# ml-unito/PartitionedLS.jl

Measured on AMD Instinct MI355X. Metric: sign-pattern NNLS solves/sec (whole node); fp64 obj gap vs ref, higher is better.
Workload: dtype f64

## Files before the change

### partitionedls.jl_amd/csrc/ctx.h

```cpp
#pragma once
#include "common.h"
#include <chrono>
#include <functional>
#include <vector>

namespace partls {

bool runtime_gone();
struct NoCopy {
    NoCopy() = default;
    NoCopy(const NoCopy &) = delete;
    NoCopy &operator=(const NoCopy &) = delete;
};

struct DevBuf : NoCopy {
    void *p = nullptr;
    size_t bytes = 0;
    ~DevBuf() { release(); }
    hipError_t ensure(size_t b)
    {
        if (b <= bytes && p) return hipSuccess;
        if (p) { hipError_t e = hipFree(p); p = nullptr; bytes = 0; if (e != hipSuccess) return e; }
        hipError_t e = hipMalloc(&p, b ? b : 8);
        if (e == hipSuccess) bytes = b;
        return e;
    }
    void release() { if (p && !runtime_gone()) (void)hipFree(p); p = nullptr; bytes = 0; }
    template <class T> T *as() const { return static_cast<T *>(p); }
};

struct DevChunks : NoCopy {
    std::vector<void *> v;
    ~DevChunks() { release(); }
    void release() { if (!runtime_gone()) for (void *q : v) (void)hipFree(q); v.clear(); }
    size_t size() const { return v.size(); }
    void push_back(void *q) { v.push_back(q); }
    void *operator[](size_t i) const { return v[i]; }
};

struct PinnedDoubles : NoCopy {
    double *p = nullptr;
    size_t cap = 0, n = 0, cap_prev = 0;
    ~PinnedDoubles() { release(); }
    hipError_t resize(size_t count)
    {
        if (count > cap) {
            if (p) (void)hipHostFree(p);
            p = nullptr; cap = 0;
            size_t want = count > 512 ? count : 512;
            if (want < 2 * cap_prev) want = 2 * cap_prev;
            hipError_t e = hipHostMalloc((void **)&p, want * sizeof(double), hipHostMallocDefault);
            if (e != hipSuccess) return e;
            cap = cap_prev = want;
        }
        n = count;
        return hipSuccess;
    }
    void release() { if (p && !runtime_gone()) (void)hipHostFree(p); p = nullptr; cap = n = 0; }
    double *data() const { return p; }
    size_t size() const { return n; }
    double &operator[](size_t i) const { return p[i]; }
};

template <class T> struct PinnedArray : NoCopy {
    T *p = nullptr;
    ~PinnedArray() { release(); }
    hipError_t alloc(size_t count)
    {
        release();
        const hipError_t e = hipHostMalloc((void **)&p, count * sizeof(T), hipHostMallocDefault);
        if (e != hipSuccess) p = nullptr;
        return e;
    }
    void release() { if (p && !runtime_gone()) (void)hipHostFree(p); p = nullptr; }
    operator T *() const { return p; }
};

struct UploadStaging : NoCopy {
    char *pin[8] = {};
    hipStream_t stream[4] = {};
    hipEvent_t event[8] = {};
    ~UploadStaging()
    {
        if (runtime_gone()) return;
        for (int i = 0; i < 8; ++i) { if (pin[i]) (void)hipHostFree(pin[i]); if (event[i]) (void)hipEventDestroy(event[i]); }
        for (int t = 0; t < 4; ++t) if (stream[t]) (void)hipStreamDestroy(stream[t]);
    }
};

}

struct partls_knobs {
    double tol_rel = 1e-11;
    long long chain_len = 0;
    long long grid = 0;
    int gram_S = 0, gram_cr = 0;
    int coop_rows = 0;
    bool no_coop = false;
    int reg_maxt = 18;
    bool no_staged_upload = false;
    bool no_export = false;
    bool eager_generic = false;
    int bnb_batch = 1024;
    int bnb_pool_mb = 65536;
    int bnb_wg_per_cu = 8;
    bool bnb_cold = false;
    bool lz_fault = false;
    int coop_fault = 0;
    bool no_tab_refine = false;
    bool finish_trace = false;
    bool alt_trace = false;
    bool alt_always_check = false;
    bool print_stamps = false;
    int alt_ms_max_rounds = 0;
    int max_rounds = 0;
    int rescue_max_passes = 0;
    long long alt_ms_chunk = 0;
    double kkt_tol = 1e-12;
    double near_tie_rel = 1e-13;
    double cal_wb = 1.0, cal_ws = 1.0;
    bool cv_serial = false;
    bool resample_serial = false;
    int pair = -1;
    long long top_piece = 0;
    int bit_order = 0;
    int batch_piece = 0;
};

struct partls_ctx {
    int device = 0;
    int ncu = 256;
    partls_knobs knobs;
    hipStream_t stream = nullptr;
    hipEvent_t ev0[PARTLS_T_COUNT] = {}, ev1[PARTLS_T_COUNT] = {};
    bool timed[PARTLS_T_COUNT] = {};
    double ms[PARTLS_T_COUNT] = {};

    bool prepared = false;
    int64_t N = 0, M = 0, K = 0, ldX = 0;
    double eta = 0.0;
    uint32_t flags = 0;
    bool faithful = false;
    const void *dX = nullptr;
    bool x_f32 = false;
    const double *dy = nullptr;
    partls::DevBuf ownX, ownY;
    const double *dw = nullptr, *ds = nullptr;
    partls::DevBuf ownW, ownS, wPart;
    bool multi_rank = false;
    std::vector<int64_t> P;
    std::vector<uint64_t> mask_aug;
    std::vector<uint64_t> pack;
    const uint64_t *maskTabP = nullptr;
    const int *permP = nullptr;
    int ldg = 0, chunks = 0;
    partls::DevBuf slab, G, maskAugD , scale, Tfull, T0reg, scratch, bestObj, bestSol , bestPat, counters, allOpt,
        wdev, partial, yhatD, gD, nodeCode, nodeSol, nodeObj, predX, predY, gridCtr, nodeTab, nodeBasic, altA, altGA, altHg,
        nodePiv, maskInt, allOptRef, bnbIn, bnbOut, altGersh, amsState, amsWork;
    partls::DevChunks bnbChunks;
    size_t bnbSlotBytes = 0, bnbMaxSlots = 0;
    int bnbChunkSlots = 512;
    std::vector<int> bnbFree, bnbRefs;
    std::vector<partls_ctx *> peers;
    partls::PinnedDoubles hPart, hGpart;
    partls::PinnedDoubles sweepOut, nodeOut, exportSol;
    partls::DevBuf mdlRows, mdlOut, mdlCtr;
    partls::PinnedDoubles mdlStage;
    partls::DevBuf topWork, topRows;
    partls::DevBuf rescueScratch, rescueList;
    partls::PinnedDoubles rescueStage;
    unsigned long long rescue_rescued = 0, rescue_pivots = 0, rescue_failed = 0;
    std::function<partls_status(partls_ctx *)> gram_hook;
    partls::PinnedDoubles amsHostIn, amsHostOut;
    partls::PinnedDoubles bnbHostIn, bnbHostOut;
    partls::UploadStaging up;
    double last_upload_ms = 0.0, last_upload_bytes = 0.0;
    partls::PinnedDoubles hG;
    partls::PinnedDoubles hScale;
    int n = 0, kbits = 0, T = 0;
    std::vector<int> perm;
    std::vector<uint64_t> mask_tab;
    bool use_reg = false;
    partls::BitOrder order{};
    bool order_ready = false, order_identity = true;
    std::vector<double> flip_cost;
    double tol = 0.0;
    unsigned long long last_pivots = 0, last_vetoes = 0, last_blocks = 0;
    std::vector<int64_t> near_pat;
    int64_t near_for = -1;
    std::vector<std::pair<double, int64_t>> cand;
    int64_t last_near_evaluated = 0;
    int export_wg = -1;
    double last_kkt = 0.0;
    double last_min_loo = 0.0;
    unsigned long long sweep_vetoes = 0;
    bool coop_state_valid = false;
    bool coop_fallback = false;
    partls::PinnedArray<double> hTab;
    partls::PinnedArray<int8_t> hBasic;
    size_t hTabDoubles = 0;
    bool tab_valid = false, tab_full = false;
    partls_ctx *cv_work = nullptr;
    std::vector<partls_ctx *> cv_view;
    partls::DevBuf cvG, cvBatch, cvEta;
    partls::PinnedDoubles cvHost, cvHostG;
    partls::DevBuf rsW, rsS, rsPart, rsWv;
    partls::PinnedDoubles rsHost;
    partls::DevBuf pmW, pmRanks, pmY, pmStats, pmMean;
};

namespace partls {

void t_begin(partls_ctx *c, int w);
void t_end(partls_ctx *c, int w);
void t_collect(partls_ctx *c);
inline double ms_since(std::chrono::steady_clock::time_point t0) { return std::chrono::duration<double, std::milli>(std::chrono::steady_clock::now() - t0).count(); }

partls_status ctx_prepare(partls_ctx *c, const void *X, int64_t N, int64_t M, int64_t ldX, const double *y, int x_on_device,
                          const int64_t *P, int64_t K, int64_t ldP, double eta, bool faithful, uint32_t flags, const double *w = nullptr,
                          bool x_f32 = false);
void forget_problem(partls_ctx *c);
partls_status adopt_or_upload(partls_ctx *c, const void *X, int64_t N, int64_t M, int64_t ldX, const double *y, int x_on_device, size_t esz);
partls_status prepare_weights(partls_ctx *c, const double *w, int64_t N, int on_device);
partls_status ctx_prepare_tableau(partls_ctx *c);
partls_status load_partition(partls_ctx *c, const int64_t *P, int64_t M, int64_t K, int64_t ldP);
partls_status upload_matrix(partls_ctx *c, void *dst, const void *X, int64_t N, int64_t M, int64_t ldX, size_t esz = sizeof(double));
constexpr double SWEEP_PIV_EPS = 1e-11;
inline int sweep_max_rounds(int n) { return 20 * (n + 1); }
SweepParams sweep_params(const partls_ctx *c, bool internal_order);
partls_status ensure_sweep_scratch(partls_ctx *c, int grid);
partls_status node_sweep_params(partls_ctx *c, size_t nodes, int64_t chain_len, int grid, SweepParams *p);
inline void bind_counters(SweepParams &p, unsigned long long *w) { p.n_unconverged = w; p.n_pivots = w + 1; p.n_vetoes = w + 2; }
struct SweepBlock { unsigned long long *counters; double *best_obj; int64_t *best_pat; double *second_obj; int64_t *second_pat; };
inline size_t sweep_block_words(int grid, bool runner_up) { return 4 + (runner_up ? 4 : 2) * (size_t)grid; }
inline SweepBlock sweep_block(double *base, int grid, bool runner_up)
{
    double *b = base + 4;
    const size_t g = (size_t)grid;
    return {reinterpret_cast<unsigned long long *>(base), b, reinterpret_cast<int64_t *>(b + g), runner_up ? b + 2 * g : nullptr,
            runner_up ? reinterpret_cast<int64_t *>(b + 3 * g) : nullptr};
}
void bind_sweep_block(SweepParams &p, double *base, int grid, bool runner_up);
hipError_t launch_any_sweep(partls_ctx *c, SweepParams &p, int grid, bool models = false);
partls_status calibrate_bit_order(partls_ctx *c);
bool sweep_plan(partls_ctx *c, int64_t total, int64_t *chain_len_out, int *grid_out, const char *who);
bool sweep_pairs(const partls_ctx *c, int64_t total);
int64_t reference_pattern(const partls_ctx *c, int64_t q);
void install_sweep_result(partls_ctx *c, const double *sweep_out, int grid, bool has_sol, double *bobj_out, int64_t *bpat_out);

struct CvOut {
    std::vector<double> alpha, beta, t, opt, sse;
    std::vector<int64_t> best;
    std::vector<int32_t> status;
    void assign(int64_t B, int64_t M, int64_t K);
    void deliver(int64_t B, int64_t M, int64_t K, double *alpha_out, int64_t ld_alpha, double *beta_out, int64_t ld_beta, double *t_out,
                 double *opt_out, int64_t *best_out, double *sse_out, int32_t *status_out) const;
};
struct ProblemBatch {
    int64_t B = 0, E = 1;
    const double *eta = nullptr;
    const double *G = nullptr, *hostG = nullptr;
    int64_t gs = 0;
    bool serial = false;
    const char *who = "";
    std::function<partls_status(int64_t q, int64_t bpat, int64_t unconv)> finish;
};
partls_status make_internal(partls_ctx *c, partls_ctx **slot);
partls_status cv_check_inputs(const char *who, partls_ctx *c, const double *X, int64_t N, int64_t M, int64_t ldX, const double *y,
                              const int64_t *P, int64_t K, int64_t ldP, const int64_t *fold_ptr, int64_t F, const double *eta, int64_t E);
partls_status cv_grams(partls_ctx *c, const double *X, int64_t N, int64_t M, int64_t ldX, const double *y, const double *w, int x_on_device,
                       int64_t K, const int64_t *fold_ptr, int64_t F, uint32_t flags, const char *who, int *ldg_out, int *chunks_out);
void cv_point_rows(partls_ctx *c, partls_ctx *W, const int64_t *fold_ptr, int64_t F, int64_t f);
partls_status cv_heldout_sse(partls_ctx *c, int64_t f, int64_t q, CvOut &o);
void batch_reset(partls_ctx *c, int64_t N, int64_t M, int64_t K, uint32_t flags);
partls_status batch_work_prepare(partls_ctx *c, const int64_t *P, int64_t ldP, uint32_t flags, int ldg, int chunks, const ProblemBatch &pb,
                                 int64_t cal_gram, const std::function<void(partls_ctx *)> &point_rows);
partls_status batch_calibrate(partls_ctx *c, const int64_t *P, int64_t ldP, uint32_t flags, int ldg, int chunks, const ProblemBatch &pb,
                              int64_t cal_gram, const std::function<void(partls_ctx *)> &point_rows);
partls_status batch_prepare_one(partls_ctx *c, const ProblemBatch &pb, int64_t q);
partls_status batch_pieces_begin(partls_ctx *c, const ProblemBatch &pb, size_t extra, int64_t *per_piece);
struct BatchPiece {
    int64_t q0 = 0;
    int bc = 0;
    size_t tfd = 0, t0d = 0;
    double *scale = nullptr, *tol = nullptr, *Tfull = nullptr, *T0reg = nullptr;
    double *tail = nullptr;
};
partls_status batch_piece_prepare(partls_ctx *c, const ProblemBatch &pb, int64_t q0, int bc, size_t tail_words, BatchPiece *pc);
partls_status batch_install(partls_ctx *c, const ProblemBatch &pb, const BatchPiece &pc, int j, const double *head);
partls_status batch_sweep(partls_ctx *c, const ProblemBatch &pb);
partls_status finish_model(partls_ctx *c, int64_t q, int64_t bpat, int64_t unconv, CvOut &o);
void model_weights(const partls_ctx *work, const CvOut &o, int64_t q, double *w);

partls_status solve_nodes(partls_ctx *c, const std::vector<int8_t> &codes, size_t cnt, std::vector<double> &sols,
                          std::vector<double> &obj2, unsigned long long *unconv, bool resume = false, bool want_tab = false);
partls_status solve_nodes_device(partls_ctx *c, size_t cnt, const int8_t *code, double *obj2, double *sol,
                                 unsigned long long *counters, int max_rounds);
partls_status solve_nodes_device_at(partls_ctx *c, const double *T0reg, double tol, size_t cnt, const int8_t *code, double *obj2,
                                    double *sol, unsigned long long *counters, int max_rounds);

struct AltProblems {
    int64_t B = 1, E = 1, q0 = 0;
    const double *G = nullptr;
    int64_t gs = 0;
    const double *eta = nullptr;
    const double *scale = nullptr;
    const double *T0reg = nullptr;
    size_t t0d = 0;
    const double *tol = nullptr;
    const double *yy = nullptr;
};
struct AltTables {
    double *alpha_all; int64_t ld_alpha_all; double *beta_all; int64_t ld_beta_all;
    double *t_all, *opt_all; int64_t *iters_all; int32_t *status_all;
};
struct AltWinner {
    int64_t start = -1, iters = 0;
    double opt = 0.0;
    std::vector<double> a, b, wv, hdiag;
    std::vector<int8_t> vcode;
};
partls_status alt_multistart_core(partls_ctx *c, const AltProblems *pp, double eps, int64_t T, int64_t R,
                                  const double *alpha0, int64_t ld_alpha0, const double *beta0, int64_t ld_beta0,
                                  const AltTables &tb, AltWinner *win);
partls_status alt_finish(partls_ctx *c, const std::vector<double> &a, const std::vector<double> &b, const std::vector<double> &wv,
                         const std::vector<int8_t> &vcode_last, const std::vector<double> &hdiag, const std::vector<double> &gersh,
                         double optval, int64_t iters_done, unsigned long long unconv_total,
                         double *alpha, double *beta, double *t, double *opt, int64_t *iters);
inline bool rescue_on(const partls_ctx *c) { return (c->flags & PARTLS_OPT_RESCUE_CAPPED) != 0; }
void rescue_begin_call(partls_ctx *c);
partls_status rescue_piece(partls_ctx *c, int64_t p0, int64_t cnt, double *rows, double *obj);
partls_status rescue_all_opt(partls_ctx *c, const double *obj, int64_t p0, int64_t cnt, double *all_opt);
void rescue_collect(partls_ctx *c, unsigned long long *unconv, unsigned long long *vetoes);
partls_status rescue_pattern(partls_ctx *c, uint64_t pattern, std::vector<double> &sol, double *obj2, unsigned long long *unconv);
void opt_codes(const partls_ctx *c, uint64_t pattern, std::vector<int8_t> &codes);

void unscale_solution(const partls_ctx *c, const double *sol, std::vector<double> &w);
partls_status data_pass(partls_ctx *c, const std::vector<double> &w, bool want_obj, bool want_grad, double *obj2, std::vector<double> *g,
                        const std::function<void()> &overlap);
partls_status data_objective(partls_ctx *c, const std::vector<double> &w, double *opt, std::vector<double> *grad = nullptr);
bool kkt_says_ill_conditioned(const partls_ctx *c);
double kkt_violation_data(const partls_ctx *c, const std::vector<double> &w, const std::vector<double> &g, const std::vector<int8_t> &code,
                          int *worst);
struct RefineOut { bool have = false; double obj = 0.0; std::vector<double> g; };
partls_status refine_solution(partls_ctx *c, std::vector<double> &w, bool free_intercept, int steps = 2, RefineOut *out = nullptr);
double h_reg(const partls_ctx *c, int a, int b);
partls_status check_common(partls_ctx *c, const void *X, int64_t N, int64_t M, int64_t ldX, const void *P, int64_t K, int64_t ldP);
partls_status predict_weights(const int64_t *P, int64_t M, int64_t K, int64_t ldP, const double *alpha, const double *beta, double *w);

}
```

### partitionedls.jl_amd/csrc/opt.hip

```cpp
#include "ctx.h"
#include "near_tie.h"
#include "sweep_rules.h"
#include <algorithm>
#include <chrono>
#include <cmath>
#include <cstdio>
#include <cstring>
#include <functional>
#include <thread>

namespace partls {

static bool opt_range_ok(const partls_ctx *c, const char *who)
{
    if (c->kbits <= 40) return true;
    set_error("%s: %d sign bits: the enumeration of 2^(K+1) patterns is out of range (K <= 39); fit(Alt) and fit(BnB) take up to 61 groups", who, c->kbits);
    return false;
}

static void cleanup_opt(const partls_ctx *c, const std::vector<double> &w, uint64_t pattern, double *alpha, double *beta, double *t)
{
    const int64_t M = c->M, K = c->K;
    std::vector<double> a((size_t)M, 0.0);
    for (int64_t m = 0; m < M; ++m) {
        const int f = sign_of_var(c->mask_aug[(size_t)m], pattern);
        a[(size_t)m] = (f != 0) ? w[(size_t)m] / (double)f : 0.0;
        if (a[(size_t)m] < 0.0) a[(size_t)m] = 0.0;
    }
    std::vector<double> A((size_t)K, 0.0);
    for (int64_t k = 0; k < K; ++k) {
        double s = 0.0;
        for (int64_t m = 0; m < M; ++m) s += (double)c->P[(size_t)m + (size_t)k * M] * a[(size_t)m];
        const double sk = ((pattern >> k) & 1ULL) ? 1.0 : -1.0;
        beta[k] = sk * s;
        A[(size_t)k] = (s == 0.0) ? 1.0 : s;
    }
    for (int64_t m = 0; m < M; ++m) {
        double s = 0.0;
        for (int64_t k = 0; k < K; ++k) s += (double)c->P[(size_t)m + (size_t)k * M] * a[(size_t)m] / A[(size_t)k];
        alpha[m] = s;
    }
    *t = w[(size_t)M];
}

}

using namespace partls;

extern "C" {

partls_status partls_opt_prepare(partls_ctx *c, const double *X, int64_t N, int64_t M, int64_t ldX, const double *y,
                                 int x_on_device, const int64_t *P, int64_t K, int64_t ldP, double eta, uint32_t flags)
try {
    return ctx_prepare(c, X, N, M, ldX, y, x_on_device, P, K, ldP, eta, (flags & PARTLS_OPT_FAITHFUL_INTERCEPT) != 0, flags);
}
PARTLS_ABI_GUARD

partls_status partls_opt_prepare_weighted(partls_ctx *c, const double *X, int64_t N, int64_t M, int64_t ldX, const double *y,
                                          const double *w, int x_on_device, const int64_t *P, int64_t K, int64_t ldP, double eta,
                                          uint32_t flags)
try {
    return ctx_prepare(c, X, N, M, ldX, y, x_on_device, P, K, ldP, eta, (flags & PARTLS_OPT_FAITHFUL_INTERCEPT) != 0, flags, w);
}
PARTLS_ABI_GUARD

partls_status partls_opt_prepare_f32(partls_ctx *c, const float *X, int64_t N, int64_t M, int64_t ldX, const double *y, const double *w,
                                     int x_on_device, const int64_t *P, int64_t K, int64_t ldP, double eta, uint32_t flags)
try {
    return ctx_prepare(c, X, N, M, ldX, y, x_on_device, P, K, ldP, eta, (flags & PARTLS_OPT_FAITHFUL_INTERCEPT) != 0, flags, w, true);
}
PARTLS_ABI_GUARD

int64_t partls_opt_num_patterns(const partls_ctx *c) { return (c && c->prepared && c->kbits <= 40) ? ((int64_t)1 << c->kbits) : 0; }

static partls_status sweep_second_pass(partls_ctx *c, int64_t g_begin, int64_t g_end, double *all_opt, double *bobj_io, int64_t *bpat_io,
                                       unsigned long long *unconv_io);

partls_status partls_opt_sweep(partls_ctx *c, int64_t g_begin, int64_t g_end, double *best_obj, int64_t *best_pattern,
                               double *all_opt, int64_t *n_unconverged)
try {
    if (!c || !c->prepared) { set_error("partls_opt_sweep: context not prepared"); return PARTLS_ERR_STATE; }
    if (!opt_range_ok(c, "partls_opt_sweep")) return PARTLS_ERR_UNSUPPORTED;
    const int64_t npat = (int64_t)1 << c->kbits;
    if (g_end < 0) g_end = npat;
    if (g_begin < 0 || g_begin > g_end || g_end > npat) { set_error("bad Gray-index range [%lld,%lld)", (long long)g_begin, (long long)g_end); return PARTLS_ERR_BAD_ARG; }
    if (all_opt && !c->faithful) { set_error("all_opt needs PARTLS_OPT_FAITHFUL_INTERCEPT"); return PARTLS_ERR_BAD_ARG; }
    PARTLS_HIP_CHECK(hipSetDevice(c->device));
    if (g_begin == g_end) {
        if (best_obj) *best_obj = INFINITY;
        if (best_pattern) *best_pattern = -1;
        if (n_unconverged) *n_unconverged = 0;
        return PARTLS_OK;
    }
    if (!c->order_ready) {
        partls_status st = calibrate_bit_order(c);
        if (st != PARTLS_OK) return st;
    }
    const int n = c->n;
    const int64_t total = g_end - g_begin;
    int64_t chain_len = 0;
    int grid = 0;
    if (!sweep_plan(c, total, &chain_len, &grid, "partls_opt_sweep")) return PARTLS_ERR_UNSUPPORTED;

    const size_t sweep_words = sweep_block_words(grid, true);
    PARTLS_HIP_CHECK(c->bestObj.ensure(sizeof(double) * sweep_block_words(std::max(grid, 4096), true)));
    PARTLS_HIP_CHECK(hipMemsetAsync(c->bestObj.p, 0, 4 * sizeof(unsigned long long), c->stream));
    if (all_opt) {
        PARTLS_HIP_CHECK(c->allOpt.ensure((size_t)npat * sizeof(double)));
        if (total < npat) PARTLS_HIP_CHECK(hipMemsetAsync(c->allOpt.p, 0xFF, (size_t)npat * sizeof(double), c->stream));
    }
    const partls_status ss = ensure_sweep_scratch(c, grid);
    if (ss != PARTLS_OK) return ss;

    SweepParams p = sweep_params(c, true);
    p.g_begin = g_begin; p.g_end = g_end; p.chain_len = chain_len;
    p.pair = sweep_pairs(c, total) ? 1 : 0;
    p.all_opt = all_opt ? c->allOpt.as<double>() : nullptr;
    bind_sweep_block(p, c->bestObj.as<double>(), grid, true);
    if (!c->use_reg && c->knobs.lz_fault) p.coop_fault = 77;
    c->export_wg = -1;
    if (((c->use_reg && (sweep_reg_small(c->T) || sweep_reg_exports(c->T))) || (!c->use_reg && !c->knobs.eager_generic)) && !c->knobs.no_export) {
        PARTLS_HIP_CHECK(c->bestSol.ensure((size_t)grid * n * sizeof(double)));
        p.best_sol = c->bestSol.as<double>();
        p.node_ld = n;
    }

    t_begin(c, PARTLS_T_SWEEP);
    PARTLS_HIP_CHECK(launch_any_sweep(c, p, grid));
    t_end(c, PARTLS_T_SWEEP);

    unsigned long long cnt[3] = {0, 0, 0};
    PARTLS_HIP_CHECK(c->sweepOut.resize(sweep_words));
    const double *sweep_out = c->sweepOut.data();
    PARTLS_HIP_CHECK(hipMemcpyAsync(c->sweepOut.data(), c->bestObj.p, sweep_words * sizeof(double), hipMemcpyDeviceToHost, c->stream));
    if (all_opt) {
        const void *src = c->allOpt.p;
        if (!c->order_identity) {
            PARTLS_HIP_CHECK(c->allOptRef.ensure((size_t)npat * sizeof(double)));
            PARTLS_HIP_CHECK(launch_pattern_gather(c->allOpt.as<double>(), npat, c->kbits, c->order, c->allOptRef.as<double>(), c->stream));
            src = c->allOptRef.p;
        }
        PARTLS_HIP_CHECK(hipMemcpyAsync(all_opt, src, (size_t)npat * sizeof(double), hipMemcpyDeviceToHost, c->stream));
    }
    PARTLS_HIP_CHECK(hipStreamSynchronize(c->stream));
    t_collect(c);
    std::memcpy(cnt, sweep_out, sizeof(cnt));
    if (c->knobs.print_stamps) {
        double st[32] = {0};
        if (hipMemcpy(st, c->scratch.p, sizeof(st), hipMemcpyDeviceToHost) == hipSuccess)
            fprintf(stderr, "[partls stamps] scan: pre %.0f barrier %.0f post %.0f | gather: work %.0f barrier %.0f | panel: work %.0f barrier %.0f | "
                            "update %.0f | scatter %.0f | chain-load %.0f/%.0f | pivots %llu || gather split: block setup %.0f chain %.0f rhs/myj %.0f"
                            " || workgroup 0: %.0f blocks, %.0f scans, %.0f pivots || pair walk: twin scan %.0f, solve + rows + scan %.0f\n",
                    st[9], st[10], st[0], st[12] + st[13] + st[8], st[1], st[11], st[2], st[3], st[4], st[5], st[6], cnt[1], st[12], st[13], st[8],
                    st[24], st[25], st[26], st[15], st[14]);
    }
    double bobj = INFINITY;
    int64_t bpat = -1;
    install_sweep_result(c, sweep_out, grid, p.best_sol != nullptr, &bobj, &bpat);
    if (rescue_on(c)) {
        rescue_begin_call(c);
        if (cnt[0]) {
            const partls_status rs = sweep_second_pass(c, g_begin, g_end, all_opt, &bobj, &bpat, &cnt[0]);
            if (rs != PARTLS_OK) return rs;
        }
    }
    if (best_obj) *best_obj = bobj;
    if (best_pattern) *best_pattern = bpat;
    if (n_unconverged) *n_unconverged = (int64_t)cnt[0];
    return PARTLS_OK;
}
PARTLS_ABI_GUARD

partls_status partls_opt_finish(partls_ctx *c, int64_t pattern, double *alpha, double *beta, double *t, double *opt,
                                int64_t *best_index)
try {
    if (!c || !c->prepared) { set_error("partls_opt_finish: context not prepared"); return PARTLS_ERR_STATE; }
    if (!alpha || !beta || !t || !opt) { set_error("partls_opt_finish: NULL output"); return PARTLS_ERR_BAD_ARG; }
    if (pattern < 0 || pattern >= ((int64_t)1 << (c->K + 1))) { set_error("pattern out of range"); return PARTLS_ERR_BAD_ARG; }
    PARTLS_HIP_CHECK(hipSetDevice(c->device));
    const uint64_t kmask = ((uint64_t)1 << c->kbits) - 1;
    uint64_t used = 1ULL << c->K;
    for (int i = 0; i < c->n; ++i) if (c->hScale[(size_t)i] != 0.0) used |= c->mask_tab[(size_t)i];

    std::vector<uint64_t> cands{(uint64_t)pattern & kmask & used};
    if (pattern == c->near_for)
        for (int64_t q : c->near_pat) {
            const uint64_t v = (uint64_t)q & kmask & used;
            if (std::find(cands.begin(), cands.end(), v) == cands.end()) cands.push_back(v);
        }
    const int export_wg = (pattern == c->near_for) ? c->export_wg : -1;
    c->export_wg = -1;
    c->near_for = -1;
    c->near_pat.clear();
    c->last_near_evaluated = (int64_t)cands.size();

    t_begin(c, PARTLS_T_FINISH);
    const auto f0 = std::chrono::steady_clock::now();
    std::vector<double> sols, obj2, w, wbest, g, gbest;
    std::vector<int8_t> codes;
    unsigned long long unconv = 0, unconv_best = 0;
    double obest = INFINITY, loo_best = 0.0;
    uint64_t pbest = cands[0];
    for (size_t ci = 0; ci < cands.size(); ++ci) {
        partls_status st = PARTLS_OK;
        bool taken = false;
        if (ci == 0 && export_wg >= 0) {
            PARTLS_HIP_CHECK(c->exportSol.resize((size_t)c->n));
            PARTLS_HIP_CHECK(hipMemcpyAsync(c->exportSol.data(), c->bestSol.as<double>() + (size_t)export_wg * c->n, (size_t)c->n * sizeof(double), hipMemcpyDeviceToHost, c->stream));
            PARTLS_HIP_CHECK(hipStreamSynchronize(c->stream));
            sols.assign(c->exportSol.data(), c->exportSol.data() + c->n);
            opt_codes(c, cands[ci], codes);
            taken = true;
            double smax = 0.0;
            for (int i = 0; i < c->n; ++i) smax = std::max(smax, std::fabs(sols[(size_t)i]));
            for (int i = 0; i < c->n && taken; ++i) {
                const double v = sols[(size_t)i];
                if (!std::isfinite(v)) taken = false;
                else if (v != 0.0 && (codes[(size_t)i] == 0 || (codes[(size_t)i] == 1 && v < -1e-9 * smax) || (codes[(size_t)i] == -1 && v > 1e-9 * smax))) taken = false;
            }
            if (taken) { c->tab_valid = false; unconv = 0; }
            if (c->knobs.finish_trace) fprintf(stderr, "[finish] the sweep's solution of its winner (workgroup %d): %s\n", export_wg, taken ? "taken" : "refused (signs), solving again");
        }
        if (!taken) {
            opt_codes(c, cands[ci], codes);
            st = solve_nodes(c, codes, 1, sols, obj2, &unconv, false, true);
            if (st != PARTLS_OK) return st;
            if (unconv && rescue_on(c)) {
                st = rescue_pattern(c, cands[ci], sols, nullptr, &unconv);
                if (st != PARTLS_OK) return st;
                c->tab_valid = false;
            }
        }
        unscale_solution(c, sols.data(), w);
        RefineOut ro;
        st = refine_solution(c, w, !c->faithful, 2, &ro);
        if (st != PARTLS_OK) return st;
        double o = 0.0;
        if (ro.have) { o = ro.obj; g.swap(ro.g); }
        else { st = data_objective(c, w, &o, &g); if (st != PARTLS_OK) return st; }
        if (c->knobs.finish_trace && cands.size() > 1) fprintf(stderr, "[finish] near tie: pattern %llu data objective %.17g\n", (unsigned long long)cands[ci], o);
        if (ci == 0 || o < obest || (o == obest && cands[ci] < pbest)) { obest = o; pbest = cands[ci]; wbest = w; gbest = g; unconv_best = unconv; loo_best = c->last_min_loo; }
    }
    const auto f1 = std::chrono::steady_clock::now();
    uint64_t full = pbest;
    if (!c->faithful) { if (wbest[(size_t)c->M] > 0.0) full |= (1ULL << c->K); }
    full &= used;
    std::vector<int8_t> vcode((size_t)c->M + 1, 0);
    for (int64_t m = 0; m <= c->M; ++m) {
        if (m == c->M && !c->faithful) { vcode[(size_t)m] = 2; continue; }
        const int f = sign_of_var(c->mask_aug[(size_t)m], full);
        vcode[(size_t)m] = (int8_t)((f > 0) - (f < 0));
    }
    int worst = -1;
    c->last_kkt = kkt_violation_data(c, wbest, gbest, vcode, &worst);
    *opt = obest;
    if (c->knobs.finish_trace) {
        const auto f2 = std::chrono::steady_clock::now();
        auto ms = [](auto a, auto b) { return std::chrono::duration<double, std::milli>(b - a).count(); };
        fprintf(stderr, "[finish] %zu candidate(s): solve + refine + data objective / gradient %.3f ms, KKT check %.3f ms; data-space KKT violation %.3e (variable %d)\n",
                cands.size(), ms(f0, f1), ms(f1, f2), c->last_kkt, worst);
    }
    t_end(c, PARTLS_T_FINISH);
    PARTLS_HIP_CHECK(hipStreamSynchronize(c->stream));
    t_collect(c);
    cleanup_opt(c, wbest, full, alpha, beta, t);
    if (best_index) *best_index = (int64_t)full;
    if (unconv_best) { set_error("winner re-solve hit the pivot cap"); return PARTLS_ERR_NOT_CONVERGED; }
    c->last_min_loo = loo_best;
    if (kkt_says_ill_conditioned(c)) {
        set_error("the winner's KKT conditions do not hold in data space (violation %.2e of ||x|| ||y|| at variable %d, tolerance %.1e; %llu columns "
                  "refused as dependent in the sweep): X is too ill-conditioned for the fp64 Gram form (cond(X) >~ 1e6); the outputs hold the best "
                  "Gram-form model", c->last_kkt, worst, c->knobs.kkt_tol, c->sweep_vetoes);
        return PARTLS_ERR_ILL_CONDITIONED;
    }
    return PARTLS_OK;
}
PARTLS_ABI_GUARD

partls_status partls_opt_pattern(partls_ctx *c, int64_t pattern, double *raw_alpha, double *optval)
try {
    if (!c || !c->prepared) { set_error("partls_opt_pattern: context not prepared"); return PARTLS_ERR_STATE; }
    if (!c->faithful) { set_error("partls_opt_pattern needs a context prepared with PARTLS_OPT_FAITHFUL_INTERCEPT"); return PARTLS_ERR_STATE; }
    if (pattern < 0 || pattern >= ((int64_t)1 << c->kbits)) { set_error("pattern out of range"); return PARTLS_ERR_BAD_ARG; }
    PARTLS_HIP_CHECK(hipSetDevice(c->device));
    std::vector<double> sols, obj2, w;
    unsigned long long unconv = 0;
    std::vector<int8_t> codes;
    opt_codes(c, (uint64_t)pattern, codes);
    partls_status st = solve_nodes(c, codes, 1, sols, obj2, &unconv, false, true);
    if (st != PARTLS_OK) return st;
    if (unconv && rescue_on(c)) {
        st = rescue_pattern(c, (uint64_t)pattern, sols, nullptr, &unconv);
        if (st != PARTLS_OK) return st;
        c->tab_valid = false;
    }
    unscale_solution(c, sols.data(), w);
    st = refine_solution(c, w, false);
    if (st != PARTLS_OK) return st;
    if (optval) { st = data_objective(c, w, optval); if (st != PARTLS_OK) return st; }
    if (raw_alpha)
        for (int64_t m = 0; m <= c->M; ++m) {
            const int f = sign_of_var(c->mask_aug[(size_t)m], (uint64_t)pattern);
            const double a = (f != 0) ? w[(size_t)m] / (double)f : 0.0;
            raw_alpha[m] = a > 0.0 ? a : 0.0;
        }
    if (unconv) { set_error("pattern solve hit the pivot cap"); return PARTLS_ERR_NOT_CONVERGED; }
    return PARTLS_OK;
}
PARTLS_ABI_GUARD

static void par_rows(int64_t rows, size_t row_bytes, const std::function<void(int64_t, int64_t)> &fn)
{
    const int nt = (size_t)rows * row_bytes < ((size_t)32 << 20) ? 1 : 8;
    if (nt == 1) { fn(0, rows); return; }
    std::vector<std::thread> th;
    const int64_t per = (rows + nt - 1) / nt;
    try {
        for (int i = 1; i < nt; ++i) {
            const int64_t r0 = std::min<int64_t>(rows, i * per), r1 = std::min<int64_t>(rows, r0 + per);
            th.emplace_back(fn, r0, r1);
        }
    } catch (...) {
        const int64_t done_from = (int64_t)(th.size() + 1) * per;
        fn(std::min<int64_t>(rows, done_from), rows);
    }
    fn(0, std::min<int64_t>(rows, per));
    for (std::thread &t : th) t.join();
}

static void copy_rows(double *dst, int64_t ld_dst, const double *src, int64_t width, int64_t rows)
{
    if (!dst || width <= 0) return;
    par_rows(rows, (size_t)width * sizeof(double), [&](int64_t r0, int64_t r1) {
        if (ld_dst == width) std::memcpy(dst + (size_t)r0 * width, src + (size_t)r0 * width, (size_t)(r1 - r0) * width * sizeof(double));
        else for (int64_t r = r0; r < r1; ++r) std::memcpy(dst + (size_t)r * ld_dst, src + (size_t)r * width, (size_t)width * sizeof(double));
    });
}

static partls_status export_begin(partls_ctx *c, const char *who, int64_t g_begin, int64_t *g_end_io, const int64_t *pattern,
                                  const double *raw_alpha, int64_t ld_raw, const double *alpha, int64_t ld_alpha, const double *beta,
                                  int64_t ld_beta, const double *t, int64_t *n_unconverged, int64_t *n_vetoes, bool *empty)
{
    if (!c || !c->prepared) { set_error("%s: context not prepared", who); return PARTLS_ERR_STATE; }
    if (!c->faithful) { set_error("%s needs a context prepared with PARTLS_OPT_FAITHFUL_INTERCEPT", who); return PARTLS_ERR_STATE; }
    if (!opt_range_ok(c, who)) return PARTLS_ERR_UNSUPPORTED;
    const int64_t npat = (int64_t)1 << c->kbits, M = c->M, K = c->K;
    int64_t g_end = *g_end_io;
    if (g_end < 0) g_end = npat;
    if (g_begin < 0 || g_begin > g_end || g_end > npat) { set_error("%s: bad Gray-index range [%lld,%lld)", who, (long long)g_begin, (long long)g_end); return PARTLS_ERR_BAD_ARG; }
    if (!pattern) { set_error("%s: pattern is NULL", who); return PARTLS_ERR_BAD_ARG; }
    if ((alpha || beta || t) && !(alpha && beta && t)) { set_error("%s: alpha, beta and t go together (all three or none)", who); return PARTLS_ERR_BAD_ARG; }
    if ((raw_alpha && ld_raw < M + 1) || (alpha && (ld_alpha < M || ld_beta < K))) { set_error("%s: leading dimension too small", who); return PARTLS_ERR_BAD_ARG; }
    if (n_unconverged) *n_unconverged = 0;
    if (n_vetoes) *n_vetoes = 0;
    PARTLS_HIP_CHECK(hipSetDevice(c->device));
    *g_end_io = g_end;
    *empty = g_begin == g_end;
    if (*empty) return PARTLS_OK;
    if (!c->order_ready) {
        partls_status st = calibrate_bit_order(c);
        if (st != PARTLS_OK) return st;
    }
    return PARTLS_OK;
}

static partls_status export_piece(partls_ctx *c, int64_t p0, int64_t cnt, double *rows, double *obj, const char *who)
{
    int64_t chain_len = 0;
    int grid = 0;
    if (!sweep_plan(c, cnt, &chain_len, &grid, who)) return PARTLS_ERR_UNSUPPORTED;
    PARTLS_HIP_CHECK(c->mdlCtr.ensure(sizeof(double) * sweep_block_words(grid, false)));
    PARTLS_HIP_CHECK(hipMemsetAsync(c->mdlCtr.p, 0, 4 * sizeof(unsigned long long), c->stream));
    const partls_status ss = ensure_sweep_scratch(c, grid);
    if (ss != PARTLS_OK) return ss;
    SweepParams p = sweep_params(c, true);
    p.g_begin = p0; p.g_end = p0 + cnt; p.chain_len = chain_len;
    bind_sweep_block(p, c->mdlCtr.as<double>(), grid, false);
    p.node_sol = rows; p.node_obj2 = obj; p.node_ld = c->n;
    PARTLS_HIP_CHECK(launch_any_sweep(c, p, grid, true));
    return PARTLS_OK;
}

static int64_t models_piece(const partls_ctx *c, int64_t total)
{
    const size_t out_w = 3 + (size_t)c->M + (size_t)c->K;
    const size_t per_pat = (size_t)c->n + 1 + out_w;
    const int64_t cap = std::max<int64_t>(1, (int64_t)(PARTLS_OPT_MODELS_PIECE_BYTES / (per_pat * sizeof(double))));
    const int64_t npieces = (total + cap - 1) / cap;
    return (total + npieces - 1) / npieces;
}

static partls_status sweep_second_pass(partls_ctx *c, int64_t g_begin, int64_t g_end, double *all_opt, double *bobj_io, int64_t *bpat_io,
                                       unsigned long long *unconv_io)
{
    const auto w0 = std::chrono::steady_clock::now();
    const int n = c->n;
    const int64_t npat = (int64_t)1 << c->kbits, total = g_end - g_begin, piece = models_piece(c, total);
    const int64_t K4 = 4, kmax = std::min<int64_t>(K4, piece);
    PARTLS_HIP_CHECK(c->mdlRows.ensure((size_t)piece * (n + 1) * sizeof(double)));
    PARTLS_HIP_CHECK(c->topWork.ensure(topk_work_bytes(kmax)));
    PARTLS_HIP_CHECK(c->topRows.ensure((size_t)kmax * (n + 2) * sizeof(double)));
    PARTLS_HIP_CHECK(c->mdlStage.resize(8 + 2 * (size_t)kmax));
    if (!c->use_reg) c->coop_state_valid = false;
    std::vector<std::pair<double, int64_t>> all;
    unsigned long long unconv = 0, pivots = 0, vetoes = 0;
    for (int64_t p0 = g_begin; p0 < g_end; p0 += piece) {
        const int64_t cnt = std::min<int64_t>(piece, g_end - p0), kk = std::min<int64_t>(K4, cnt);
        double *rows = c->mdlRows.as<double>(), *obj = rows + (size_t)cnt * n;
        double *crow = c->topRows.as<double>(), *cobj = crow + (size_t)kk * n;
        int64_t *glist = reinterpret_cast<int64_t *>(cobj + kk);
        partls_status st = export_piece(c, p0, cnt, rows, obj, "partls_opt_sweep");
        if (st == PARTLS_OK) st = rescue_piece(c, p0, cnt, rows, obj);
        if (st == PARTLS_OK && all_opt) st = rescue_all_opt(c, obj, p0, cnt, c->allOpt.as<double>());
        if (st != PARTLS_OK) return st;
        PARTLS_HIP_CHECK(launch_topk_select(obj, cnt, p0, K4, c->kbits, c->order, c->order_identity, c->topWork.p, c->stream));
        PARTLS_HIP_CHECK(launch_topk_gather(rows, obj, n, p0, cnt, kk, c->topWork.p, crow, cobj, glist, c->stream));
        const TopkWork w = topk_work(c->topWork.p, kk);
        double *hs = c->mdlStage.data();
        PARTLS_HIP_CHECK(hipMemcpyAsync(hs, c->mdlCtr.p, 4 * sizeof(double), hipMemcpyDeviceToHost, c->stream));
        PARTLS_HIP_CHECK(hipMemcpyAsync(hs + 4, c->topWork.p, 4 * sizeof(double), hipMemcpyDeviceToHost, c->stream));
        PARTLS_HIP_CHECK(hipMemcpyAsync(hs + 8, cobj, (size_t)kk * sizeof(double), hipMemcpyDeviceToHost, c->stream));
        PARTLS_HIP_CHECK(hipMemcpyAsync(hs + 8 + kk, w.out_pat, (size_t)kk * sizeof(int64_t), hipMemcpyDeviceToHost, c->stream));
        PARTLS_HIP_CHECK(hipStreamSynchronize(c->stream));
        unsigned long long cn[8];
        std::memcpy(cn, hs, sizeof(cn));
        unsigned long long left = cn[0], vet = cn[2];
        rescue_collect(c, &left, &vet);
        unconv += left; pivots += cn[1]; vetoes += vet;
        const int64_t got = (int64_t)cn[7];
        if (got < 0 || got > kk) { set_error("partls_opt_sweep: the selection reported %lld rows of at most %lld", (long long)got, (long long)kk); return PARTLS_ERR_HIP; }
        for (int64_t i = 0; i < got; ++i) {
            int64_t pat = 0;
            std::memcpy(&pat, hs + 8 + kk + i, sizeof(pat));
            all.emplace_back(hs[8 + i], pat);
        }
    }
    if (all_opt) {
        const void *src = c->allOpt.p;
        if (!c->order_identity) {
            PARTLS_HIP_CHECK(c->allOptRef.ensure((size_t)npat * sizeof(double)));
            PARTLS_HIP_CHECK(launch_pattern_gather(c->allOpt.as<double>(), npat, c->kbits, c->order, c->allOptRef.as<double>(), c->stream));
            src = c->allOptRef.p;
        }
        PARTLS_HIP_CHECK(hipMemcpyAsync(all_opt, src, (size_t)npat * sizeof(double), hipMemcpyDeviceToHost, c->stream));
        PARTLS_HIP_CHECK(hipStreamSynchronize(c->stream));
    }
    c->last_pivots += pivots + c->rescue_pivots;
    c->last_vetoes += vetoes;
    c->sweep_vetoes += vetoes;
    c->export_wg = -1;
    c->near_pat.clear();
    c->cand.clear();
    c->near_for = -1;
    double bobj = INFINITY;
    int64_t bpat = -1;
    if (!all.empty()) {
        const std::pair<double, int64_t> win = *std::min_element(all.begin(), all.end());
        bobj = win.first; bpat = win.second;
        const double yy = h_reg(c, (int)c->M + 1, (int)c->M + 1);
        const double lim2 = bobj * bobj + c->knobs.near_tie_rel * (yy > 0.0 ? yy : 0.0);
        install_near_ties(win, std::move(all), lim2, 3, c->cand, c->near_pat, c->near_for);
    }
    *bobj_io = bobj; *bpat_io = bpat; *unconv_io = unconv;
    c->ms[PARTLS_T_SWEEP] += std::chrono::duration<double, std::milli>(std::chrono::steady_clock::now() - w0).count();
    return PARTLS_OK;
}

partls_status partls_opt_models(partls_ctx *c, int64_t g_begin, int64_t g_end, int64_t *pattern, double *optval, double *raw_alpha,
                                int64_t ld_raw, double *alpha, int64_t ld_alpha, double *beta, int64_t ld_beta, double *t,
                                int64_t *n_unconverged, int64_t *n_vetoes)
try {
    bool empty = false;
    const partls_status bs = export_begin(c, "partls_opt_models", g_begin, &g_end, pattern, raw_alpha, ld_raw, alpha, ld_alpha, beta, ld_beta, t,
                                          n_unconverged, n_vetoes, &empty);
    if (bs != PARTLS_OK || empty) return bs;
    const int64_t M = c->M, K = c->K;
    const int n = c->n;
    const int64_t total = g_end - g_begin;
    const size_t out_w = 3 + (size_t)M + (size_t)K;
    const int64_t piece = models_piece(c, total);
    PARTLS_HIP_CHECK(c->mdlRows.ensure((size_t)piece * (n + 1) * sizeof(double)));
    PARTLS_HIP_CHECK(c->mdlOut.ensure((size_t)piece * out_w * sizeof(double)));
    const size_t stage_words = 4 + (size_t)piece * (out_w + (raw_alpha ? (size_t)n : 0));
    PARTLS_HIP_CHECK(c->mdlStage.resize(stage_words));
    if (!c->use_reg) c->coop_state_valid = false;
    const bool rescue = rescue_on(c);
    if (rescue) rescue_begin_call(c);
    unsigned long long unconv = 0, vetoes = 0;
    for (int64_t p0 = g_begin; p0 < g_end; p0 += piece) {
        const int64_t cnt = std::min<int64_t>(piece, g_end - p0);
        double *rows = c->mdlRows.as<double>(), *obj = rows + (size_t)cnt * n, *out = c->mdlOut.as<double>();
        partls_status es = export_piece(c, p0, cnt, rows, obj, "partls_opt_models");
        if (es == PARTLS_OK && rescue) es = rescue_piece(c, p0, cnt, rows, obj);
        if (es != PARTLS_OK) return es;
        PARTLS_HIP_CHECK(launch_models_cleanup(rows, obj, p0, cnt, (int)M, (int)K, c->kbits, c->order, c->order_identity, c->permP,
                                               c->scale.as<double>(), c->maskAugD.as<uint64_t>(), raw_alpha != nullptr, out, c->stream));
        double *st = c->mdlStage.data();
        PARTLS_HIP_CHECK(hipMemcpyAsync(st, c->mdlCtr.p, 4 * sizeof(double), hipMemcpyDeviceToHost, c->stream));
        PARTLS_HIP_CHECK(hipMemcpyAsync(st + 4, out, (size_t)cnt * out_w * sizeof(double), hipMemcpyDeviceToHost, c->stream));
        if (raw_alpha) PARTLS_HIP_CHECK(hipMemcpyAsync(st + 4 + (size_t)cnt * out_w, rows, (size_t)cnt * n * sizeof(double), hipMemcpyDeviceToHost, c->stream));
        PARTLS_HIP_CHECK(hipStreamSynchronize(c->stream));
        unsigned long long cn[3];
        std::memcpy(cn, st, sizeof(cn));
        if (rescue) rescue_collect(c, &cn[0], &cn[2]);
        unconv += cn[0];
        vetoes += cn[2];
        const double *o = st + 4;
        const size_t r = (size_t)(p0 - g_begin);
        std::memcpy(pattern + r, o, (size_t)cnt * sizeof(int64_t));
        if (optval) std::memcpy(optval + r, o + cnt, (size_t)cnt * sizeof(double));
        if (t) std::memcpy(t + r, o + 2 * cnt, (size_t)cnt * sizeof(double));
        if (alpha) {
            copy_rows(alpha + r * ld_alpha, ld_alpha, o + 3 * cnt, M, cnt);
            copy_rows(beta + r * ld_beta, ld_beta, o + 3 * cnt + (size_t)cnt * M, K, cnt);
        }
        if (raw_alpha) copy_rows(raw_alpha + r * ld_raw, ld_raw, o + (size_t)cnt * out_w, M + 1, cnt);
    }
    if (n_unconverged) *n_unconverged = (int64_t)unconv;
    if (n_vetoes) *n_vetoes = (int64_t)vetoes;
    return PARTLS_OK;
}
PARTLS_ABI_GUARD

static bool top_before(double oa, int64_t pa, double ob, int64_t pb) { return oa < ob || (oa == ob && pa < pb); }

partls_status partls_opt_top(partls_ctx *c, int64_t g_begin, int64_t g_end, int64_t k, int64_t *pattern, double *optval, double *raw_alpha,
                             int64_t ld_raw, double *alpha, int64_t ld_alpha, double *beta, int64_t ld_beta, double *t, int64_t *count,
                             int64_t *n_unconverged, int64_t *n_vetoes)
try {
    bool empty = false;
    const partls_status bs = export_begin(c, "partls_opt_top", g_begin, &g_end, pattern, raw_alpha, ld_raw, alpha, ld_alpha, beta, ld_beta, t,
                                          n_unconverged, n_vetoes, &empty);
    if (bs != PARTLS_OK) return bs;
    if (!optval || !count) { set_error("partls_opt_top: optval or count is NULL"); return PARTLS_ERR_BAD_ARG; }
    if (k < 1 || k > PARTLS_OPT_TOP_MAX_K) { set_error("partls_opt_top: k = %lld outside 1 .. %d", (long long)k, PARTLS_OPT_TOP_MAX_K); return PARTLS_ERR_BAD_ARG; }
    *count = 0;
    if (empty) return PARTLS_OK;
    const int64_t M = c->M, K = c->K;
    const int n = c->n;
    const int64_t total = g_end - g_begin;
    const size_t out_w = 3 + (size_t)M + (size_t)K;
    int64_t cap = std::max<int64_t>(1, (int64_t)(PARTLS_OPT_MODELS_PIECE_BYTES / (((size_t)n + 1) * sizeof(double))));
    if (c->knobs.top_piece > 0) cap = (int64_t)c->knobs.top_piece;
    cap = std::min<int64_t>(cap, (int64_t)1 << 30);
    const int64_t npieces = (total + cap - 1) / cap;
    const int64_t piece = (total + npieces - 1) / npieces;
    const int64_t kmax = std::min<int64_t>(k, piece);
    PARTLS_HIP_CHECK(c->mdlRows.ensure((size_t)piece * (n + 1) * sizeof(double)));
    PARTLS_HIP_CHECK(c->mdlOut.ensure((size_t)kmax * out_w * sizeof(double)));
    PARTLS_HIP_CHECK(c->topWork.ensure(topk_work_bytes(kmax)));
    PARTLS_HIP_CHECK(c->topRows.ensure((size_t)kmax * (n + 2) * sizeof(double)));
    const size_t stage_words = 8 + (size_t)kmax * (out_w + (raw_alpha ? (size_t)n : 0));
    PARTLS_HIP_CHECK(c->mdlStage.resize(stage_words));
    if (!c->use_reg) c->coop_state_valid = false;
    const bool rescue = rescue_on(c);
    if (rescue) rescue_begin_call(c);
    unsigned long long unconv = 0, vetoes = 0;
    const size_t roww = 3 + (alpha ? (size_t)(M + K) : 0) + (raw_alpha ? (size_t)n : 0);
    std::vector<double> best, next;
    int64_t nbest = 0;
    for (int64_t p0 = g_begin; p0 < g_end; p0 += piece) {
        const int64_t cnt = std::min<int64_t>(piece, g_end - p0), kk = std::min<int64_t>(k, cnt);
        double *rows = c->mdlRows.as<double>(), *obj = rows + (size_t)cnt * n, *out = c->mdlOut.as<double>();
        double *crow = c->topRows.as<double>(), *cobj = crow + (size_t)kk * n;
        int64_t *glist = reinterpret_cast<int64_t *>(cobj + kk);
        partls_status es = export_piece(c, p0, cnt, rows, obj, "partls_opt_top");
        if (es == PARTLS_OK && rescue) es = rescue_piece(c, p0, cnt, rows, obj);
        if (es != PARTLS_OK) return es;
        PARTLS_HIP_CHECK(launch_topk_select(obj, cnt, p0, k, c->kbits, c->order, c->order_identity, c->topWork.p, c->stream));
        PARTLS_HIP_CHECK(launch_topk_gather(rows, obj, n, p0, cnt, kk, c->topWork.p, crow, cobj, glist, c->stream));
        PARTLS_HIP_CHECK(launch_models_cleanup(crow, cobj, p0, kk, (int)M, (int)K, c->kbits, c->order, c->order_identity, c->permP,
                                               c->scale.as<double>(), c->maskAugD.as<uint64_t>(), raw_alpha != nullptr, out, c->stream, glist));
        double *st = c->mdlStage.data();
        PARTLS_HIP_CHECK(hipMemcpyAsync(st, c->mdlCtr.p, 4 * sizeof(double), hipMemcpyDeviceToHost, c->stream));
        PARTLS_HIP_CHECK(hipMemcpyAsync(st + 4, c->topWork.p, 4 * sizeof(double), hipMemcpyDeviceToHost, c->stream));
        PARTLS_HIP_CHECK(hipMemcpyAsync(st + 8, out, (size_t)kk * out_w * sizeof(double), hipMemcpyDeviceToHost, c->stream));
        if (raw_alpha) PARTLS_HIP_CHECK(hipMemcpyAsync(st + 8 + (size_t)kk * out_w, crow, (size_t)kk * n * sizeof(double), hipMemcpyDeviceToHost, c->stream));
        PARTLS_HIP_CHECK(hipStreamSynchronize(c->stream));
        unsigned long long cn[8];
        std::memcpy(cn, st, sizeof(cn));
        if (rescue) rescue_collect(c, &cn[0], &cn[2]);
        unconv += cn[0];
        vetoes += cn[2];
        const int64_t got = (int64_t)cn[7];
        if (got < 0 || got > kk) { set_error("partls_opt_top: the selection reported %lld rows of at most %lld", (long long)got, (long long)kk); return PARTLS_ERR_HIP; }
        const double *o = st + 8;
        const int64_t *opat = reinterpret_cast<const int64_t *>(o);
        const double *oopt = o + kk, *ot = o + 2 * kk, *oal = o + 3 * kk, *obe = oal + (size_t)kk * M, *oraw = o + (size_t)kk * out_w;
        const int64_t keep = std::min<int64_t>(k, nbest + got);
        next.resize((size_t)keep * roww);
        int64_t ia = 0, ib = 0;
        for (int64_t r = 0; r < keep; ++r) {
            double *d = next.data() + (size_t)r * roww;
            const double *a = best.data() + (size_t)ia * roww;
            int64_t apat = 0;
            if (ia < nbest) std::memcpy(&apat, a + 1, sizeof(apat));
            const bool take_a = ia < nbest && (ib >= got || top_before(a[0], apat, oopt[ib], opat[ib]));
            if (take_a) { std::memcpy(d, a, roww * sizeof(double)); ++ia; continue; }
            d[0] = oopt[ib];
            std::memcpy(d + 1, &opat[ib], sizeof(int64_t));
            d[2] = ot[ib];
            double *e = d + 3;
            if (alpha) {
                std::memcpy(e, oal + (size_t)ib * M, (size_t)M * sizeof(double));
                std::memcpy(e + M, obe + (size_t)ib * K, (size_t)K * sizeof(double));
                e += M + K;
            }
            if (raw_alpha) std::memcpy(e, oraw + (size_t)ib * n, (size_t)n * sizeof(double));
            ++ib;
        }
        best.swap(next);
        nbest = keep;
    }
    for (int64_t r = 0; r < nbest; ++r) {
        const double *d = best.data() + (size_t)r * roww, *e = d + 3;
        optval[r] = d[0];
        std::memcpy(&pattern[r], d + 1, sizeof(int64_t));
        if (alpha) {
            t[r] = d[2];
            std::memcpy(alpha + (size_t)r * ld_alpha, e, (size_t)M * sizeof(double));
            std::memcpy(beta + (size_t)r * ld_beta, e + M, (size_t)K * sizeof(double));
            e += M + K;
        }
        if (raw_alpha) std::memcpy(raw_alpha + (size_t)r * ld_raw, e, (size_t)n * sizeof(double));
    }
    *count = nbest;
    if (n_unconverged) *n_unconverged = (int64_t)unconv;
    if (n_vetoes) *n_vetoes = (int64_t)vetoes;
    return PARTLS_OK;
}
PARTLS_ABI_GUARD

partls_status partls_opt_top_select(partls_ctx *c, const double *obj, int64_t cnt, int64_t g0, int64_t k, int64_t *index, int64_t *pattern,
                                    double *optval, int64_t *count)
try {
    if (!c || !c->prepared) { set_error("partls_opt_top_select: context not prepared"); return PARTLS_ERR_STATE; }
    if (!opt_range_ok(c, "partls_opt_top_select")) return PARTLS_ERR_UNSUPPORTED;
    if (!obj || !index || !pattern || !optval || !count) { set_error("partls_opt_top_select: NULL argument"); return PARTLS_ERR_BAD_ARG; }
    if (k < 1 || k > PARTLS_OPT_TOP_MAX_K) { set_error("partls_opt_top_select: k = %lld outside 1 .. %d", (long long)k, PARTLS_OPT_TOP_MAX_K); return PARTLS_ERR_BAD_ARG; }
    const int64_t npat = (int64_t)1 << c->kbits;
    if (cnt < 0 || cnt >= ((int64_t)1 << 31) || g0 < 0 || g0 > npat || cnt > npat - g0) { set_error("partls_opt_top_select: bad range g0 = %lld, cnt = %lld", (long long)g0, (long long)cnt); return PARTLS_ERR_BAD_ARG; }
    *count = 0;
    PARTLS_HIP_CHECK(hipSetDevice(c->device));
    if (cnt == 0) return PARTLS_OK;
    if (!c->order_ready) {
        partls_status st = calibrate_bit_order(c);
        if (st != PARTLS_OK) return st;
    }
    const int64_t kk = std::min<int64_t>(k, cnt);
    PARTLS_HIP_CHECK(c->mdlRows.ensure((size_t)cnt * sizeof(double)));
    PARTLS_HIP_CHECK(c->topWork.ensure(topk_work_bytes(kk)));
    PARTLS_HIP_CHECK(c->mdlStage.resize(4 + 2 * (size_t)kk));
    PARTLS_HIP_CHECK(hipMemcpyAsync(c->mdlRows.p, obj, (size_t)cnt * sizeof(double), hipMemcpyHostToDevice, c->stream));
    PARTLS_HIP_CHECK(launch_topk_select(c->mdlRows.as<double>(), cnt, g0, k, c->kbits, c->order, c->order_identity, c->topWork.p, c->stream));
    const TopkWork w = topk_work(c->topWork.p, kk);
    double *st = c->mdlStage.data();
    PARTLS_HIP_CHECK(hipMemcpyAsync(st, c->topWork.p, 4 * sizeof(double), hipMemcpyDeviceToHost, c->stream));
    PARTLS_HIP_CHECK(hipMemcpyAsync(st + 4, w.out_idx, 2 * (size_t)kk * sizeof(int64_t), hipMemcpyDeviceToHost, c->stream));
    PARTLS_HIP_CHECK(hipStreamSynchronize(c->stream));
    unsigned long long hd[4];
    std::memcpy(hd, st, sizeof(hd));
    const int64_t got = (int64_t)hd[3];
    if (got < 0 || got > kk) { set_error("partls_opt_top_select: the selection reported %lld rows of at most %lld", (long long)got, (long long)kk); return PARTLS_ERR_HIP; }
    std::memcpy(index, st + 4, (size_t)got * sizeof(int64_t));
    std::memcpy(pattern, st + 4 + kk, (size_t)got * sizeof(int64_t));
    for (int64_t i = 0; i < got; ++i) {
        if (index[i] < 0 || index[i] >= cnt) { set_error("partls_opt_top_select: selected position out of range"); return PARTLS_ERR_HIP; }
        optval[i] = obj[index[i]];
    }
    *count = got;
    return PARTLS_OK;
}
PARTLS_ABI_GUARD

partls_status partls_fit_opt(partls_ctx *c, const double *X, int64_t N, int64_t M, int64_t ldX, const double *y,
                             const int64_t *P, int64_t K, int64_t ldP, double eta, uint32_t flags,
                             double *alpha, double *beta, double *t, double *opt, int64_t *best_index, double *all_opt)
try {
    if (all_opt) flags |= PARTLS_OPT_FAITHFUL_INTERCEPT;
    partls_status st = partls_opt_prepare(c, X, N, M, ldX, y, 0, P, K, ldP, eta, flags);
    if (st != PARTLS_OK) return st;
    double bobj; int64_t bpat, unconv;
    st = partls_opt_sweep(c, 0, -1, &bobj, &bpat, all_opt, &unconv);
    if (st != PARTLS_OK) return st;
    if (bpat < 0) { set_error("sweep produced no candidate"); return PARTLS_ERR_NOT_CONVERGED; }
    st = partls_opt_finish(c, bpat, alpha, beta, t, opt, best_index);
    if (st != PARTLS_OK) return st;
    if (unconv) { set_error("%lld subproblems hit the pivot cap", (long long)unconv); return PARTLS_ERR_NOT_CONVERGED; }
    return PARTLS_OK;
}
PARTLS_ABI_GUARD

partls_status partls_opt_bit_order(partls_ctx *c, int64_t *gbit, double *flip_cost)
try {
    if (!c || !c->prepared) { set_error("partls_opt_bit_order: context not prepared"); return PARTLS_ERR_STATE; }
    if (!gbit) { set_error("partls_opt_bit_order: gbit is NULL"); return PARTLS_ERR_BAD_ARG; }
    if (!opt_range_ok(c, "partls_opt_bit_order")) return PARTLS_ERR_UNSUPPORTED;
    PARTLS_HIP_CHECK(hipSetDevice(c->device));
    if (!c->order_ready) {
        partls_status st = calibrate_bit_order(c);
        if (st != PARTLS_OK) return st;
    }
    for (int k = 0; k < c->kbits; ++k) {
        gbit[k] = c->order.gbit[k];
        if (flip_cost) flip_cost[k] = c->flip_cost.empty() ? -1.0 : c->flip_cost[(size_t)k];
    }
    return PARTLS_OK;
}
PARTLS_ABI_GUARD

partls_status partls_opt_candidates(const partls_ctx *c, int64_t capacity, double *obj, int64_t *pattern, int64_t *count)
try {
    if (!c || !c->prepared || !count || capacity < 0 || (capacity > 0 && (!obj || !pattern))) { set_error("partls_opt_candidates: bad argument"); return PARTLS_ERR_BAD_ARG; }
    const int64_t n = std::min<int64_t>(capacity, (int64_t)c->cand.size());
    for (int64_t i = 0; i < n; ++i) { obj[i] = c->cand[(size_t)i].first; pattern[i] = c->cand[(size_t)i].second; }
    *count = n;
    return PARTLS_OK;
}
PARTLS_ABI_GUARD

partls_status partls_opt_merge_candidates(partls_ctx *c, int64_t count, const double *obj, const int64_t *pattern, double *win_obj, int64_t *win_pattern)
try {
    if (!c || !c->prepared || count < 0 || (count > 0 && (!obj || !pattern))) { set_error("partls_opt_merge_candidates: bad argument"); return PARTLS_ERR_BAD_ARG; }
    std::vector<std::pair<double, int64_t>> all;
    for (int64_t i = 0; i < count; ++i) if (pattern[i] >= 0 && obj[i] == obj[i]) all.emplace_back(obj[i], pattern[i]);
    const int64_t local_winner = c->cand.empty() ? -1 : c->cand[0].second;
    c->near_pat.clear();
    c->cand.clear();
    if (all.empty()) { c->near_for = -1; c->export_wg = -1; if (win_obj) *win_obj = INFINITY; if (win_pattern) *win_pattern = -1; return PARTLS_OK; }
    const std::pair<double, int64_t> win = *std::min_element(all.begin(), all.end());
    const double bobj = win.first;
    const int64_t bpat = win.second;
    const double yy = h_reg(c, (int)c->M + 1, (int)c->M + 1);
    const double lim2 = bobj * bobj + c->knobs.near_tie_rel * (yy > 0.0 ? yy : 0.0);
    install_near_ties(win, std::move(all), lim2, 3, c->cand, c->near_pat, c->near_for);
    if (local_winner != bpat) c->export_wg = -1;
    if (win_obj) *win_obj = bobj;
    if (win_pattern) *win_pattern = bpat;
    return PARTLS_OK;
}
PARTLS_ABI_GUARD

}
```

### partitionedls.jl_amd/csrc/prepare.hip

```cpp
#include "ctx.h"
#include "prepare_rules.h"
#include <algorithm>
#include <chrono>
#include <cmath>
#include <cstring>
#include <numeric>
#include <thread>

namespace partls {

partls_status load_partition(partls_ctx *c, const int64_t *P, int64_t M, int64_t K, int64_t ldP)
{
    c->P.assign((size_t)M * K, 0);
    c->mask_aug.assign((size_t)M + 2, 0);
    for (int64_t k = 0; k < K; ++k)
        for (int64_t m = 0; m < M; ++m) {
            const int64_t v = P[m + k * ldP];
            if (v != 0 && v != 1) { set_error("P[%lld,%lld] = %lld is not 0/1", (long long)m, (long long)k, (long long)v); return PARTLS_ERR_BAD_PARTITION; }
            c->P[(size_t)m + (size_t)k * M] = v;
            if (v) c->mask_aug[(size_t)m] |= (1ULL << k);
        }
    c->mask_aug[(size_t)M] = 1ULL << K;
    c->mask_aug[(size_t)M + 1] = 0;
    return PARTLS_OK;
}

namespace {
constexpr int UP_T = 4;
constexpr size_t UP_BUF = (size_t)8 << 20;
}
partls_status upload_matrix(partls_ctx *c, void *dst_, const void *X_, int64_t N, int64_t M, int64_t ldX, size_t esz)
{
    char *dst = static_cast<char *>(dst_);
    const char *X = static_cast<const char *>(X_);
    const size_t bytes = (size_t)N * M * esz;
    if (bytes < ((size_t)8 << 20) || c->knobs.no_staged_upload) {
        PARTLS_HIP_CHECK(hipMemcpy2DAsync(dst, (size_t)N * esz, X, (size_t)ldX * esz, (size_t)N * esz, (size_t)M,
                                          hipMemcpyHostToDevice, c->stream));
        return PARTLS_OK;
    }
    if (!c->up.pin[0]) {
        for (int i = 0; i < 2 * UP_T; ++i) PARTLS_HIP_CHECK(hipHostMalloc((void **)&c->up.pin[i], UP_BUF, hipHostMallocDefault));
        for (int t = 0; t < UP_T; ++t) PARTLS_HIP_CHECK(hipStreamCreateWithFlags(&c->up.stream[t], hipStreamNonBlocking));
        for (int i = 0; i < 2 * UP_T; ++i) PARTLS_HIP_CHECK(hipEventCreateWithFlags(&c->up.event[i], hipEventDisableTiming));
    }
    const size_t col_bytes = (size_t)N * esz, ld_bytes = (size_t)ldX * esz;
    hipError_t err[UP_T];
    for (int t = 0; t < UP_T; ++t) err[t] = hipSuccess;
    const int device = c->device;
    auto worker = [&](int t) {
        hipError_t e = hipSetDevice(device);
        const int64_t c0 = M * t / UP_T, c1 = M * (t + 1) / UP_T;
        char *pin[2] = {c->up.pin[2 * t], c->up.pin[2 * t + 1]};
        bool used[2] = {false, false};
        int b = 0;
        auto flush = [&](char *d, size_t n) {
            if (e == hipSuccess) e = hipMemcpyAsync(d, pin[b], n, hipMemcpyHostToDevice, c->up.stream[t]);
            if (e == hipSuccess) e = hipEventRecord(c->up.event[2 * t + b], c->up.stream[t]);
            used[b] = true;
            b ^= 1;
            if (used[b] && e == hipSuccess) e = hipEventSynchronize(c->up.event[2 * t + b]);
        };
        if (col_bytes <= UP_BUF) {
            const int64_t per = (int64_t)(UP_BUF / col_bytes);
            for (int64_t j0 = c0; j0 < c1 && e == hipSuccess; j0 += per) {
                const int64_t j1 = j0 + per < c1 ? j0 + per : c1;
                for (int64_t j = j0; j < j1; ++j) std::memcpy(pin[b] + (size_t)(j - j0) * col_bytes, X + (size_t)j * ld_bytes, col_bytes);
                flush(dst + (size_t)j0 * col_bytes, (size_t)(j1 - j0) * col_bytes);
            }
        } else {
            const int64_t rows = (int64_t)(UP_BUF / esz);
            for (int64_t j = c0; j < c1 && e == hipSuccess; ++j)
                for (int64_t r0 = 0; r0 < N && e == hipSuccess; r0 += rows) {
                    const int64_t r1 = r0 + rows < N ? r0 + rows : N;
                    std::memcpy(pin[b], X + (size_t)j * ld_bytes + (size_t)r0 * esz, (size_t)(r1 - r0) * esz);
                    flush(dst + (size_t)j * col_bytes + (size_t)r0 * esz, (size_t)(r1 - r0) * esz);
                }
        }
        if (e == hipSuccess) e = hipStreamSynchronize(c->up.stream[t]);
        err[t] = e;
    };
    {
        std::vector<std::thread> th;
        th.reserve(UP_T);
        bool spawned = true;
        try { for (int t = 1; t < UP_T; ++t) th.emplace_back(worker, t); }
        catch (...) { spawned = false; }
        worker(0);
        for (std::thread &w : th) w.join();
        if (!spawned) for (int t = (int)th.size() + 1; t < UP_T; ++t) worker(t);
    }
    PARTLS_HIP_CHECK(hipSetDevice(c->device));
    for (int t = 0; t < UP_T; ++t) if (err[t] != hipSuccess) { set_error("staged upload of X failed: %s", hipGetErrorString(err[t])); return PARTLS_ERR_HIP; }
    return PARTLS_OK;
}

partls_status prepare_weights(partls_ctx *c, const double *w, int64_t N, int on_device)
{
    c->dw = nullptr; c->ds = nullptr;
    const double *dw = w;
    if (!on_device) {
        PARTLS_HIP_CHECK(c->ownW.ensure((size_t)N * sizeof(double)));
        PARTLS_HIP_CHECK(hipMemcpyAsync(c->ownW.p, w, (size_t)N * sizeof(double), hipMemcpyHostToDevice, c->stream));
        dw = c->ownW.as<double>();
    }
    const int nb = weight_prep_blocks(N);
    PARTLS_HIP_CHECK(c->ownS.ensure((size_t)N * sizeof(double)));
    PARTLS_HIP_CHECK(c->wPart.ensure((size_t)4 * nb * sizeof(double)));
    PARTLS_HIP_CHECK(c->hPart.resize((size_t)4 * nb));
    PARTLS_HIP_CHECK(launch_weight_prep(dw, N, c->ownS.as<double>(), c->wPart.as<double>(), c->stream));
    PARTLS_HIP_CHECK(hipMemcpyAsync(c->hPart.data(), c->wPart.p, (size_t)4 * nb * sizeof(double), hipMemcpyDeviceToHost, c->stream));
    PARTLS_HIP_CHECK(hipStreamSynchronize(c->stream));
    const WeightFold f = fold_weight_partials(c->hPart.data(), nb);
    if (f.nonfinite) { set_error("the sample weights contain NaN/Inf"); return PARTLS_ERR_NONFINITE; }
    if (f.negative) { set_error("a sample weight is negative"); return PARTLS_ERR_BAD_ARG; }
    if (!(f.sum > 0.0)) { set_error("the sample weights sum to 0"); return PARTLS_ERR_BAD_ARG; }
    if (!std::isfinite(f.sum)) { set_error("the sum of the sample weights overflows"); return PARTLS_ERR_NONFINITE; }
    c->dw = dw; c->ds = c->ownS.as<double>();
    return PARTLS_OK;
}

void forget_problem(partls_ctx *c)
{
    c->prepared = false;
    c->peers.clear();
    c->near_for = -1; c->near_pat.clear(); c->cand.clear(); c->export_wg = -1;
    c->sweep_vetoes = 0;
    c->rescue_rescued = c->rescue_pivots = c->rescue_failed = 0;
    c->coop_state_valid = false; c->coop_fallback = false;
    c->tab_valid = false;
    c->order_ready = false; c->order_identity = true; c->flip_cost.clear();
    c->dw = nullptr; c->ds = nullptr;
    c->x_f32 = false;
    c->last_upload_ms = 0.0; c->last_upload_bytes = 0.0;
    c->ms[PARTLS_T_CALIB] = 0.0; c->ms[PARTLS_T_OOB] = 0.0;
}

partls_status adopt_or_upload(partls_ctx *c, const void *X, int64_t N, int64_t M, int64_t ldX, const double *y, int x_on_device, size_t esz)
{
    if (x_on_device) {
        c->dX = X; c->dy = y; c->ldX = ldX;
        return PARTLS_OK;
    }
    PARTLS_HIP_CHECK(c->ownX.ensure((size_t)N * M * esz));
    PARTLS_HIP_CHECK(c->ownY.ensure((size_t)N * sizeof(double)));
    PARTLS_HIP_CHECK(hipMemcpyAsync(c->ownY.p, y, (size_t)N * sizeof(double), hipMemcpyHostToDevice, c->stream));
    const auto u0 = std::chrono::steady_clock::now();
    const partls_status st = upload_matrix(c, c->ownX.p, X, N, M, ldX, esz);
    if (st != PARTLS_OK) return st;
    c->last_upload_ms = std::chrono::duration<double, std::milli>(std::chrono::steady_clock::now() - u0).count();
    c->last_upload_bytes = (double)N * (double)M * (double)esz;
    c->dX = c->ownX.p; c->dy = c->ownY.as<double>(); c->ldX = N;
    return PARTLS_OK;
}

partls_status ctx_prepare(partls_ctx *c, const void *X, int64_t N, int64_t M, int64_t ldX, const double *y, int x_on_device,
                          const int64_t *P, int64_t K, int64_t ldP, double eta, bool faithful, uint32_t flags, const double *w, bool x_f32)
{
    partls_status st = check_common(c, X, N, M, ldX, P, K, ldP);
    if (st != PARTLS_OK) return st;
    if (!y) { set_error("y is NULL"); return PARTLS_ERR_BAD_ARG; }
    if (!(eta >= 0.0)) { set_error("eta must be >= 0"); return PARTLS_ERR_BAD_ARG; }
    forget_problem(c);
    if (x_f32 && c->multi_rank) { set_error("float X: a context of a partls_multi is not supported (row-sharded multi-GPU fits are fp64)"); return PARTLS_ERR_UNSUPPORTED; }
    PARTLS_HIP_CHECK(hipSetDevice(c->device));
    if (w) {
        if (c->multi_rank) { set_error("sample weights: a context of a partls_multi is not supported (multi-GPU fits are unweighted)"); return PARTLS_ERR_UNSUPPORTED; }
        st = prepare_weights(c, w, N, x_on_device);
        if (st != PARTLS_OK) return st;
    }
    st = load_partition(c, P, M, K, ldP);
    if (st != PARTLS_OK) return st;
    c->N = N; c->M = M; c->K = K; c->eta = eta; c->flags = flags; c->faithful = faithful;

    st = adopt_or_upload(c, X, N, M, ldX, y, x_on_device, x_f32 ? sizeof(float) : sizeof(double));
    if (st != PARTLS_OK) return st;
    c->x_f32 = x_f32;

    const size_t slabd = gram_slab_doubles(N, M, c->knobs.gram_S, c->knobs.gram_cr, &c->chunks, &c->ldg);
    PARTLS_HIP_CHECK(c->slab.ensure(slabd * sizeof(double)));
    PARTLS_HIP_CHECK(c->G.ensure((size_t)c->ldg * c->ldg * sizeof(double)));
    t_begin(c, PARTLS_T_GRAM);
    PARTLS_HIP_CHECK(launch_gram(c->dX, N, M, c->ldX, c->dy, c->slab.as<double>(), c->chunks, c->ldg, c->knobs.gram_S, c->knobs.gram_cr,
                                 c->G.as<double>(), c->stream, c->ds, c->x_f32));
    t_end(c, PARTLS_T_GRAM);
    if (c->gram_hook) { st = c->gram_hook(c); if (st != PARTLS_OK) return st; }
    return ctx_prepare_tableau(c);
}

partls_status ctx_prepare_tableau(partls_ctx *c)
{
    const int64_t M = c->M, K = c->K;
    const double eta = c->eta;
    const bool faithful = c->faithful;
    const uint32_t flags = c->flags;
    c->n = faithful ? (int)M + 1 : (int)M;
    c->kbits = faithful ? (int)K + 1 : (int)K;
    c->perm.resize((size_t)c->n);
    std::iota(c->perm.begin(), c->perm.end(), 0);
    auto key = [&](int v) { const uint64_t m = c->mask_aug[(size_t)v]; return m ? __builtin_ctzll(m) : 64; };
    std::stable_sort(c->perm.begin(), c->perm.end(), [&](int a, int b) { return key(a) < key(b); });
    c->mask_tab.resize((size_t)c->n);
    for (int i = 0; i < c->n; ++i) c->mask_tab[(size_t)i] = c->mask_aug[(size_t)c->perm[(size_t)i]];

    {
        const size_t words = (size_t)M + 2 + (size_t)c->n + ((size_t)c->n + 1) / 2;
        c->pack.assign(words, 0);
        std::memcpy(c->pack.data(), c->mask_aug.data(), ((size_t)M + 2) * sizeof(uint64_t));
        std::memcpy(c->pack.data() + M + 2, c->mask_tab.data(), (size_t)c->n * sizeof(uint64_t));
        std::memcpy(c->pack.data() + M + 2 + c->n, c->perm.data(), (size_t)c->n * sizeof(int));
        PARTLS_HIP_CHECK(c->maskAugD.ensure(words * sizeof(uint64_t)));
        PARTLS_HIP_CHECK(hipMemcpyAsync(c->maskAugD.p, c->pack.data(), words * sizeof(uint64_t), hipMemcpyHostToDevice, c->stream));
        c->maskTabP = c->maskAugD.as<uint64_t>() + M + 2;
        c->permP = reinterpret_cast<int *>(c->maskAugD.as<uint64_t>() + M + 2 + c->n);
    }
    PARTLS_HIP_CHECK(c->scale.ensure((size_t)c->n * sizeof(double)));
    PARTLS_HIP_CHECK(c->Tfull.ensure((size_t)(c->n + 1) * (c->n + 1) * sizeof(double)));
    t_begin(c, PARTLS_T_PREP);
    PARTLS_HIP_CHECK(launch_prep(c->G.as<double>(), c->ldg, (int)M, eta, c->maskAugD.as<uint64_t>(), faithful ? 0 : 1,
                                 c->permP, c->scale.as<double>(), c->Tfull.as<double>(), c->n, c->stream));
    c->use_reg = sweep_reg_supported(c->n) && c->n <= 16 * c->knobs.reg_maxt && !(flags & PARTLS_OPT_GENERIC_KERNEL);
    if (c->use_reg) {
        c->T = sweep_reg_tiles(c->n);
        PARTLS_HIP_CHECK(c->T0reg.ensure(sweep_reg_t0_doubles(c->T) * sizeof(double)));
        PARTLS_HIP_CHECK(launch_layout_reg(c->Tfull.as<double>(), c->n, c->T, c->T0reg.as<double>(), c->stream));
    }
    t_end(c, PARTLS_T_PREP);
    PARTLS_HIP_CHECK(c->hG.resize((size_t)c->ldg * c->ldg));
    PARTLS_HIP_CHECK(c->hScale.resize((size_t)c->n));
    PARTLS_HIP_CHECK(hipMemcpyAsync(c->hG.data(), c->G.p, c->hG.size() * sizeof(double), hipMemcpyDeviceToHost, c->stream));
    PARTLS_HIP_CHECK(hipMemcpyAsync(c->hScale.data(), c->scale.p, (size_t)c->n * sizeof(double), hipMemcpyDeviceToHost, c->stream));
    PARTLS_HIP_CHECK(hipStreamSynchronize(c->stream));
    t_collect(c);
    if (!gram_diag_finite(c->hG.data(), c->ldg, M)) { set_error("X or y contains NaN/Inf (or overflows in X'X)"); return PARTLS_ERR_NONFINITE; }
    c->tol = problem_tol(c->knobs.tol_rel, c->hG[(size_t)(M + 1) * c->ldg + (M + 1)]);
    c->prepared = true;
    return PARTLS_OK;
}

}
```

### partitionedls.jl_amd/csrc/sweep_blk.hip

```cpp
#include "sweep_rules.h"
#include <atomic>
#include <type_traits>

namespace partls {
namespace blk {

static constexpr int THREADS = 512;
static constexpr int MAXT = 20;
#ifndef PARTLS_UPD_UNROLL
#define PARTLS_UPD_UNROLL 1
#endif
static constexpr int MB = 8;
#ifndef PARTLS_EXPORT_BIG
#define PARTLS_EXPORT_BIG 1
#endif
#ifndef PARTLS_MERGED_SCAN
#define PARTLS_MERGED_SCAN 1
#endif
#ifndef PARTLS_LANE_MASKS
#define PARTLS_LANE_MASKS 1
#endif
#ifndef PARTLS_MB_BIG
#define PARTLS_MB_BIG 8
#endif
#ifndef PARTLS_PAIR
#define PARTLS_PAIR 1
#endif
static constexpr int EXPORT_MAXT = 17;
static constexpr int MBB = PARTLS_MB_BIG;
static constexpr int NO_VETO = 99;
static constexpr int PAIR_MAXC = 16;
static constexpr int PAIR_PIV_MIN_HI = 0x3f1a36e2;
static constexpr int F64_EXP_HI = 0x7ff00000;

constexpr int nslots(int T) { return T * (T + 1) / 2; }
constexpr int tri(int g) { return g * (g + 1) / 2; }
constexpr int split(int T)
{
    int best = 1, bestmax = 1 << 30;
    for (int g = 1; g < T; ++g) {
        int a = tri(g), b = nslots(T) - tri(g);
        int m = a > b ? a : b;
        if (m < bestmax) { bestmax = m; best = g; }
    }
    return T == 1 ? 1 : best;
}
constexpr int rstride(int T) { return (T % 2) ? T : T + 1; }
constexpr int colw(int T) { return 513; }
static constexpr int MAXT_S = 10;
static constexpr int CW_S = 257;
template <class PT> __device__ __forceinline__ PT *uniform_ptr(PT *p)
{
    const unsigned long long v = (unsigned long long)p;
    const unsigned lo = (unsigned)__builtin_amdgcn_readfirstlane((int)v), hi = (unsigned)__builtin_amdgcn_readfirstlane((int)(v >> 32));
    return (PT *)(((unsigned long long)hi << 32) | lo);
}

#ifdef PARTLS_STAMPS
#define STAMP_DECL unsigned long long st_acc[24] = {0, 0, 0, 0, 0, 0, 0, 0, 0, 0, 0, 0, 0, 0, 0, 0, 0, 0, 0, 0, 0, 0, 0, 0}; unsigned long long st_t = __builtin_amdgcn_s_memtime();
#define STAMP(ph) do { __builtin_amdgcn_sched_barrier(0); unsigned long long _n = __builtin_amdgcn_s_memtime(); \
                       st_acc[ph] += _n - st_t; st_t = _n; __builtin_amdgcn_sched_barrier(0); } while (0)
#ifndef PARTLS_STAMP_TID
#define PARTLS_STAMP_TID 0
#endif
#define STAMP_FLUSH do { if (tid == PARTLS_STAMP_TID && blockIdx.x == 0 && p.scratch) { for (int _i = 0; _i < 24; ++_i) p.scratch[_i] = (double)st_acc[_i]; \
                                p.scratch[24] = (double)bc; p.scratch[25] = (double)sc; p.scratch[26] = (double)npiv; } } while (0)
#else
#define STAMP_DECL
#define STAMP(ph) do { } while (0)
#define STAMP_FLUSH do { } while (0)
#endif

static constexpr int CWMAX = colw(MAXT);
template <int CWX, int MAXTX>
struct LdsImageT {
    double Z[MB * CWX];
    double U[2 * (MB + 64)];
    double Dinv[MB + 64];
    unsigned long long s_inf[32];
    unsigned long long s_bas[16];
    unsigned long long s_sum[16];
    int s_veto[2];
    double s_best[4];
    unsigned char s_rbit[64];
    unsigned long long s_vmask[16 * MAXTX];
    double Pbase[2 * MB * CWX];
};
struct LdsImage {
    double Z[MBB * CWMAX];
    double U[2 * (MBB + 64)];
    double Dinv[MBB + 64];
    unsigned long long s_inf[32];
    unsigned long long s_bas[16];
    unsigned long long s_sum[16];
    int s_veto[2];
    double s_best[4];
    unsigned char s_rbit[64];
    unsigned long long s_vmask[16 * MAXT];
    double Pbase[2 * MBB * CWMAX];
};
static_assert(2 * MBB >= PAIR_MAXC, "the pair walk gathers up to PAIR_MAXC columns into the two panel buffers");
__shared__ LdsImage lds_image;
__shared__ LdsImageT<CW_S, MAXT_S> lds_small;

template <int W>
__device__ __forceinline__ auto *image_of()
{
    if constexpr (W == 1) return &lds_small; else return &lds_image;
}

template <int T, int H, int W = 2>
struct Half {
    static constexpr int G = W == 1 ? T : split(T);
    static constexpr int GLO = H ? G : 0;
    static constexpr int GHI = H ? T : G;
    static constexpr int OFF = H ? tri(G) : 0;
    static constexpr int CNT = (H ? nslots(T) - tri(G) : tri(G)) > 0 ? (H ? nslots(T) - tri(G) : tri(G)) : 1;
    static constexpr int XN = GHI;
    static constexpr int RS = rstride(T);
    static constexpr int CW = W == 1 ? CW_S : colw(T);
    static constexpr int NT = W == 1 ? 256 : THREADS;
    __device__ static constexpr int idx(int rho, int gam) { return tri(gam) + rho - OFF; }
};

template <class L>
__device__ __forceinline__ void tiles_store(double *dst, const double (&S)[L::CNT], int t8)
{
    double *bp = uniform_ptr(dst) + (size_t)L::OFF * 256;
#pragma unroll
    for (int s = 0; s < L::CNT; ++s) {
        if ((s & 1) == 0) asm volatile("" : "+s"(bp));
        bp[(s & 1) * 256 + t8] = S[s];
        if (s & 1) bp += 512;
    }
}

template <int T, int H, int W, int KAPPA, class SA>
__device__ __forceinline__ void gather_tile(const SA &S, double *P, int a, int b, unsigned pm)
{
    using L = Half<T, H, W>;
    if constexpr (KAPPA >= L::GLO && KAPPA < L::GHI) {
        if ((pm >> b) & 1u) {
            double *col = P + __builtin_popcount(pm & ((1u << b) - 1u)) * L::CW + a * L::RS;
#pragma unroll
            for (int rho = 0; rho <= KAPPA; ++rho) col[rho] = S[L::idx(rho, KAPPA)];
        }
    }
    if ((pm >> a) & 1u) {
        double *col = P + __builtin_popcount(pm & ((1u << a) - 1u)) * L::CW + b * L::RS;
#pragma unroll
        for (int gam = (KAPPA + 1 > L::GLO ? KAPPA + 1 : L::GLO); gam < L::GHI; ++gam) col[gam] = S[L::idx(KAPPA, gam)];
    }
}

template <int T, int H, int W, int KAPPA, class SA>
__device__ __forceinline__ void scatter_tile(SA &S, const double *P, int a, int b, unsigned pm)
{
    using L = Half<T, H, W>;
    if constexpr (KAPPA >= L::GLO && KAPPA < L::GHI) {
        if ((pm >> b) & 1u) {
            const double *col = P + __builtin_popcount(pm & ((1u << b) - 1u)) * L::CW + a * L::RS;
#pragma unroll
            for (int rho = 0; rho <= KAPPA; ++rho) S[L::idx(rho, KAPPA)] = col[rho];
        }
    }
    if ((pm >> a) & 1u) {
        const double *col = P + __builtin_popcount(pm & ((1u << a) - 1u)) * L::CW + b * L::RS;
#pragma unroll
        for (int gam = (KAPPA > L::GLO ? KAPPA : L::GLO); gam < L::GHI; ++gam) S[L::idx(KAPPA, gam)] = col[gam];
    }
}

template <int M, int CW, int MBK>
__device__ __forceinline__ int panel_block(double *P, double *Z, double *U, double *Dinv, int myj, bool my_basic,
                                           double piv_eps, int tid, int prow, bool idle_wave)
{
    if (idle_wave) {
#pragma unroll
        for (int s = 0; s < M; ++s) __syncthreads();
        return M;
    }
    constexpr int US = MBK + 64;
    const int dummy = MBK + (tid & 63);
    double pv[M];
#pragma unroll
    for (int j = 0; j < M; ++j) pv[j] = P[j * CW + prow];
    const int uslot = myj >= 0 ? myj : dummy;
    int veto = M;
#pragma unroll
    for (int s = 0; s < M; ++s) {
        Z[s * CW + prow] = pv[s];
        U[(s & 1) * US + uslot] = pv[s];
        if (myj == s) {
            const double d = pv[s];
            Dinv[s] = (my_basic || d > piv_eps) ? rcp_newton(d) : 0.0;
        }
        __syncthreads();
        double inv = Dinv[s];
        double u[M];
#pragma unroll
        for (int j = 0; j < M; ++j) u[j] = U[(s & 1) * US + j];
        asm volatile("" : "+v"(inv));
#pragma unroll
        for (int j = 0; j < M; ++j) asm volatile("" : "+v"(u[j]));
        if ((pv[s] * pv[s]) * (inv * piv_eps) >= 1.0) veto = veto < s ? veto : s;
        if (__builtin_amdgcn_readfirstlane(__double2hiint(inv)) & 0x7ff00000) {
            const double ainv = fabs(inv), fz = -pv[s] * inv;
            if (myj == s) {
#pragma unroll
                for (int j = 0; j < M; ++j) pv[j] = (j == s) ? -inv : u[j] * ainv;
            } else {
#pragma unroll
                for (int j = 0; j < M; ++j) pv[j] = (j == s) ? pv[s] * ainv : fma(fz, u[j], pv[j]);
            }
        }
    }
#pragma unroll
    for (int j = 0; j < M; ++j) P[j * CW + prow] = pv[j];
    return veto;
}

template <int CW>
__device__ __forceinline__ void pair_solve(const double *P, const int *cpos, int m, int lane, int rhspos, double *out)
{
    const int r = lane & 15, h = lane >> 4;
    const int code = cpos[r < m ? r : 0];
    const unsigned basm = (unsigned)__ballot(code < 0 && lane < m);
    const int pos = code < 0 ? ~code : code;
    double pv[4];
#pragma unroll
    for (int jj = 0; jj < 4; ++jj) {
        const int c = 4 * h + jj;
        const double v = P[c * CW + pos];
        pv[jj] = (r < m && c < m) ? v : 0.0;
    }
    double qc = P[r * CW + rhspos];
    if (r >= m) qc = 0.0;
    bool hard = false;
#pragma unroll 1
    for (int s = 0; s < m; ++s) {
        const double d = readlane_f64(pv[0], s);
        const int dh = __double2hiint(d);
        if ((!((basm >> s) & 1u) && !(dh > PAIR_PIV_MIN_HI)) || (dh & F64_EXP_HI) == F64_EXP_HI) { hard = true; break; }
        const double inv = rcp_newton(d), ainv = fabs(inv);
        const double pvs = __shfl(pv[0], r);
        const double fz = -pvs * inv;
        const double qs = readlane_f64(qc, s);
        double val[4];
#pragma unroll
        for (int jj = 0; jj < 4; ++jj) {
            const double u = __shfl(pv[0], (s + 4 * h + jj) & 15);
            val[jj] = (r == s) ? u * ainv : fma(fz, u, pv[jj]);
        }
        if (h == 0) val[0] = (r == s) ? -inv : pvs * ainv;
        qc = (r == s) ? qs * ainv : fma(fz, qs, qc);
        const double nx = __shfl(val[0], (lane + 16) & 63);
        pv[0] = val[1]; pv[1] = val[2]; pv[2] = val[3]; pv[3] = nx;
    }
    if (lane < PAIR_MAXC) {
        out[PAIR_MAXC + lane] = qc;
        out[lane] = ((basm >> lane) & 1u) ? -qc : qc;
    }
    if (lane == 0) out[2 * PAIR_MAXC + 1] = hard ? 1.0 : 0.0;
}

#define PARTLS_CASES(M) M(0) M(1) M(2) M(3) M(4) M(5) M(6) M(7) M(8) M(9) M(10) M(11) M(12) M(13) M(14) M(15) M(16) M(17) M(18) M(19)

template <int T, int H, bool NODE, int W = 2, bool MODELS = false, bool BATCH = false, bool PAIRK = false>
__device__ __forceinline__ void sweep_body(const SweepParams &p)
{
    using L = Half<T, H, W>;
    constexpr int RS = L::RS, CW = L::CW, RHSPOS = 16 * RS, NW = (T + 3) / 4;
    constexpr int THREADS = L::NT;
    constexpr int MB = W == 1 ? blk::MB : MBB;
    static_assert(!(NODE && MODELS), "node mode exports no per-pattern models (finish_pattern's capped flag is chain mode's)");
    constexpr bool MERGED = PARTLS_MERGED_SCAN && !NODE && !BATCH && T <= 17;
    constexpr bool LANE_MASKS = PARTLS_LANE_MASKS && !BATCH && T <= 16;
    constexpr bool PAIR = PAIRK && PARTLS_PAIR && MERGED && LANE_MASKS && W == 2 && !MODELS;
    static_assert(PAIR == PAIRK, "the pair walk is launched only where it is compiled (pair_compiled)");
    static_assert(W == 2 || RHSPOS < 256, "the 256-thread kernel needs every panel row position (and the rhs row) below 256");
    auto &lds_image = *image_of<W>();
    const int tid = threadIdx.x, t8 = tid & 255, a = t8 & 15, b = t8 >> 4, lane = tid & 63, wave = tid >> 6;
    const int n = p.n;
    const int nwords = (n + 63) >> 6;

    double *const Pbase = lds_image.Pbase, *const Z = lds_image.Z, *const U = lds_image.U, *const Dinv = lds_image.Dinv;
    unsigned long long *const s_inf = lds_image.s_inf, *const s_bas = lds_image.s_bas, *const s_vmask = lds_image.s_vmask;
    unsigned long long *const s_sum = lds_image.s_sum;
    int *const s_veto = lds_image.s_veto;
    double *const s_best = lds_image.s_best;
    [[maybe_unused]] double *const s_pair = U;
    [[maybe_unused]] int *const s_cpos = reinterpret_cast<int *>(Dinv);
    [[maybe_unused]] int *const s_tw = s_cpos + PAIR_MAXC;
    static_assert(2 * (MB + 64) >= 2 * PAIR_MAXC + 2, "pair_solve's `out` (doubles) fits U");
    static_assert(2 * (MB + 64) >= PAIR_MAXC + 8, "s_cpos and s_tw (PAIR_MAXC + 8 ints) fit Dinv (MB + 64 doubles)");
    for (int i = tid; i < 2 * MB * CW; i += THREADS) Pbase[i] = 0.0;
    for (int i = tid; i < MB * CW; i += THREADS) Z[i] = 0.0;
    if (tid < 2 * (MB + 64)) U[tid] = 0.0;
    if (tid < MB + 64) Dinv[tid] = 0.0;
    if (tid < 32) s_inf[tid] = 0;
    if (tid < 16) { s_bas[tid] = 0; s_sum[tid] = 0; }
    if (tid < 2) s_veto[tid] = NO_VETO;
    if (tid == 0) {
        s_best[0] = __builtin_inf(); reinterpret_cast<long long *>(s_best)[1] = -1;
        s_best[2] = __builtin_inf(); reinterpret_cast<long long *>(s_best)[3] = -1;
    }
    if (tid < 16 * T) s_vmask[tid] = tid < p.n ? p.mask[tid] : 0ULL;
    if (tid < 64) lds_image.s_rbit[tid] = tid < 40 ? p.rbit.gbit[tid] : 0;
    __syncthreads();

    double S[L::CNT];
    double q = 0.0, corner = 0.0;
    double mybest = __builtin_inf();
    const bool has_var = tid < n;
    bool basic = false, blocked = false;
    const int mypos = (tid & 15) * RS + (tid >> 4);
    const int rowc = tid / RS, rowrho = tid - rowc * RS;
    const bool idle_wave = __builtin_amdgcn_readfirstlane((tid & ~63) > RHSPOS ? 1 : 0) != 0;

    unsigned npiv = 0, nunconv = 0, nveto = 0;
    unsigned bc = 0, sc = 0;

    const int clen = (int)p.chain_len;
    const int nchains = (int)((p.g_end - p.g_begin + clen - 1) / clen);

    STAMP_DECL
    for (int chain = blockIdx.x; chain < nchains; chain += gridDim.x) {
        const int64_t g0 = p.g_begin + (int64_t)chain * clen;
        const int glen = (int)((g0 + clen < p.g_end) ? clen : p.g_end - g0);
        STAMP(5);
        const double *src = p.T0;
        if constexpr (NODE) {
            if (p.node_src) {
                const double *snap = p.node_src[chain];
                if (snap) src = snap;
            }
        }
        {
            const double *bp = uniform_ptr(src) + (size_t)L::OFF * 256;
#pragma unroll
            for (int s = 0; s < L::CNT; ++s) {
                if ((s & 1) == 0) asm volatile("" : "+s"(bp));
                S[s] = bp[(s & 1) * 256 + t8];
                if (s & 1) bp += 512;
            }
        }
        q = (tid < 16 * T) ? src[(size_t)nslots(T) * 256 + tid] : 0.0;
        corner = src[(size_t)nslots(T) * 256 + 16 * T];
        basic = false;
        if constexpr (NODE) {
            if (src != p.T0 && tid < 16 * T) basic = reinterpret_cast<const int8_t *>(src + (nslots(T) * 256 + 16 * T + 8))[tid] != 0;
        }
        STAMP(6);

        auto finish_pattern = [&](int gi, [[maybe_unused]] bool capped) {
            const uint64_t g = (uint64_t)g0 + (unsigned)gi;
            const uint64_t pat = NODE ? (uint64_t)chain : g ^ (g >> 1);
            const double obj2 = corner > 0.0 ? corner : 0.0;
            if constexpr (NODE) {
                if (p.node_piv && tid == 0) {
                    unsigned *o = p.node_piv + 3 * ((size_t)chain * clen + gi);
                    o[0] = npiv; o[1] = bc; o[2] = sc;
                }
            }
            if (p.all_opt && tid == THREADS - 1) p.all_opt[pat] = sqrt(obj2);
            if constexpr (MODELS) {
                const size_t row = (size_t)chain * (size_t)clen + (size_t)gi;
                if (has_var) p.node_sol[row * p.node_ld + tid] = capped ? __builtin_nan("") : (basic ? q : 0.0);
                if (tid == THREADS - 1) p.node_obj2[row] = capped ? __builtin_nan("") : sqrt(obj2);
            }
            if constexpr (!NODE && !MODELS && (W == 1 || (PARTLS_EXPORT_BIG && T <= EXPORT_MAXT))) {
                if (p.best_sol && obj2 < mybest) {
                    mybest = obj2;
                    if (has_var) p.best_sol[(size_t)blockIdx.x * p.node_ld + tid] = basic ? q : 0.0;
                }
            }
            if (tid == THREADS - 1 && obj2 <= s_best[2]) {
                const double bo = s_best[0];
                const long long bp = reinterpret_cast<long long *>(s_best)[1];
                if (obj2 < bo || (obj2 == bo && ref_index_less(pat, (unsigned long long)bp, lds_image.s_rbit))) {
                    s_best[2] = bo; reinterpret_cast<long long *>(s_best)[3] = bp;
                    s_best[0] = obj2; reinterpret_cast<long long *>(s_best)[1] = (long long)pat;
                } else if (obj2 < s_best[2] || ref_index_less(pat, (unsigned long long)reinterpret_cast<long long *>(s_best)[3], lds_image.s_rbit)) {
                    s_best[2] = obj2; reinterpret_cast<long long *>(s_best)[3] = (long long)pat;
                }
            }
        };
        [[maybe_unused]] auto record_twin = [&](int gi, double cornerv, double qv, bool bv) {
            const uint64_t g = (uint64_t)g0 + (unsigned)gi;
            const uint64_t pat = g ^ (g >> 1);
            const double obj2 = cornerv > 0.0 ? cornerv : 0.0;
            if (p.all_opt && tid == THREADS - 1) p.all_opt[pat] = sqrt(obj2);
            if constexpr (PARTLS_EXPORT_BIG && T <= EXPORT_MAXT) {
                if (p.best_sol && obj2 < mybest) {
                    mybest = obj2;
                    if (has_var) p.best_sol[(size_t)blockIdx.x * p.node_ld + tid] = bv ? qv : 0.0;
                }
            }
            if (tid == THREADS - 1 && obj2 <= s_best[2]) {
                const double bo = s_best[0];
                const long long bp = reinterpret_cast<long long *>(s_best)[1];
                if (obj2 < bo || (obj2 == bo && ref_index_less(pat, (unsigned long long)bp, lds_image.s_rbit))) {
                    s_best[2] = bo; reinterpret_cast<long long *>(s_best)[3] = bp;
                    s_best[0] = obj2; reinterpret_cast<long long *>(s_best)[1] = (long long)pat;
                } else if (obj2 < s_best[2] || ref_index_less(pat, (unsigned long long)reinterpret_cast<long long *>(s_best)[3], lds_image.s_rbit)) {
                    s_best[2] = obj2; reinterpret_cast<long long *>(s_best)[3] = (long long)pat;
                }
            }
        };
        int gi = 0;
        [[maybe_unused]] bool tw_pending = false;
        [[maybe_unused]] int pr_ncol = -1;
        [[maybe_unused]] auto pair_partner = [&](int i) -> int {
            const int j = (((unsigned)g0 + (unsigned)i) & 1u) ? i - 1 : i + 1;
            return (PAIR && j >= 0 && j < glen) ? j : -1;
        };
        [[maybe_unused]] auto pair_unit_end = [&](int i) -> int { const int j = pair_partner(i); return (j > i ? j : i) + 1; };
        [[maybe_unused]] auto pair_target = [&](int u, int i) -> int {
            const unsigned gu = (unsigned)g0 + (unsigned)u, gc = (unsigned)g0 + (unsigned)i;
            if (pair_partner(u) < 0 || (gu & 1u)) return u;
            return (((gu >> 1) ^ gu ^ (gc >> 1) ^ gc) & 1u) ? u + 1 : u;
        };
        [[maybe_unused]] auto pair_next = [&](bool to_twin, int &f, int &fn) -> bool {
            if (to_twin) gi = pair_partner(gi);
            else {
                const int u = pair_unit_end(gi);
                if (u >= glen) return false;
                gi = pair_target(u, gi);
            }
            tw_pending = !to_twin && pair_partner(gi) >= 0;
            const uint64_t vmask = s_vmask[tid < 16 * T ? tid : 0] & (has_var ? ~0ULL : 0ULL);
            const uint64_t g = (uint64_t)g0 + (unsigned)gi;
            f = sign_of_var(vmask, g ^ (g >> 1));
            const int u2 = pair_unit_end(gi);
            fn = f;
            if (u2 < glen) { const uint64_t gn = (uint64_t)g0 + (unsigned)pair_target(u2, gi); fn = sign_of_var(vmask, gn ^ (gn >> 1)); }
            return true;
        };
        for (;;) {
            [[maybe_unused]] const unsigned nunconv0 = nunconv;
            bool isfree = false;
            int f = 0;
            [[maybe_unused]] int fn = 0;
            if constexpr (NODE) {
                const int code = has_var ? (int)p.node_code[((size_t)chain * clen + gi) * p.node_ld + tid] : 0;
                isfree = code == 2;
                f = isfree ? 0 : code;
            } else {
                const uint64_t vmask = s_vmask[tid < 16 * T ? tid : 0] & (has_var ? ~0ULL : 0ULL);
                const uint64_t g = (uint64_t)g0 + (unsigned)gi, gn = g + 1;
                f = sign_of_var(vmask, g ^ (g >> 1));
                if constexpr (MERGED) fn = glen > 1 ? sign_of_var(vmask, gn ^ (gn >> 1)) : f;
                if constexpr (PAIR) {
                    tw_pending = pair_partner(0) >= 0;
                    const int u2 = pair_unit_end(0);
                    fn = f;
                    if (u2 < glen) { const uint64_t g2 = (uint64_t)g0 + (unsigned)pair_target(u2, 0); fn = sign_of_var(vmask, g2 ^ (g2 >> 1)); }
                }
            }
            blocked = false;
            int ninf_best = n + 1, patience = 3, rounds = 0;
            bool progress = false;
            for (;;) {
                if (progress) blocked = false;
                progress = false;
                const int par = sc & 1;
                ++sc;
                bool bad = false;
                [[maybe_unused]] bool nxt = false;
                if (has_var) {
                    const double fq = q * (double)(f > 1 ? 1 : (f < -1 ? -1 : f));
                    if (NODE && isfree) bad = !basic && !blocked && (fabs(q) > p.tol);
                    else if (basic) bad = (f == 0) || (fq < -p.tol);
                    else bad = (fq > p.tol) && !blocked;
                    if constexpr (MERGED) {
                        const double fqn = q * (double)(fn > 1 ? 1 : (fn < -1 ? -1 : fn));
                        nxt = basic ? ((fn == 0) || (fqn < -p.tol)) : (fqn > p.tol);
                    }
                }
                const unsigned long long bb = __ballot(bad), bs = __ballot(basic);
                unsigned summ = (unsigned)__popcll(bb);
#pragma unroll
                for (int sub = 0; sub < 4; ++sub)
                    if ((bb >> (16 * sub)) & 0xFFFFull) summ |= 0x100u << sub;
                if constexpr (!MERGED) {
                    if (lane == 0 && wave < nwords) { s_inf[par * 8 + wave] = bb; s_bas[par * 8 + wave] = bs; s_sum[par * 8 + wave] = summ; }
                } else {
                    const unsigned long long bn = __ballot(nxt);
                    unsigned summ2 = (unsigned)__popcll(bn);
#pragma unroll
                    for (int sub = 0; sub < 4; ++sub)
                        if ((bn >> (16 * sub)) & 0xFFFFull) summ2 |= 0x100u << sub;
                    if (lane == 0 && wave < nwords) {
                        s_inf[par * 8 + wave] = bb; s_inf[16 + par * 8 + wave] = bn; s_bas[par * 8 + wave] = bs;
                        s_sum[par * 8 + wave] = ((unsigned long long)summ2 << 32) | summ;
                    }
                }
                STAMP(9);
                __syncthreads();
                STAMP(10);
                int count = 0;
                unsigned tiles = 0;
                [[maybe_unused]] int count2 = 0;
                [[maybe_unused]] unsigned tiles2 = 0;
#pragma unroll
                for (int w = 0; w < NW; ++w) {
                    const unsigned long long sw2 = s_sum[par * 8 + w];
                    const unsigned sw = (unsigned)__builtin_amdgcn_readfirstlane((int)sw2);
                    count += (int)(sw & 0xFFu);
                    tiles |= (sw >> 8) << (4 * w);
                    if constexpr (MERGED) {
                        const unsigned sn = (unsigned)__builtin_amdgcn_readfirstlane((int)(sw2 >> 32));
                        count2 += (int)(sn & 0xFFu);
                        tiles2 |= (sn >> 8) << (4 * w);
                    }
                }
                STAMP(0);
                int soff = par * 8;
                bool all = true;
                bool done = count == 0;
                if (!done) {
                    if (count < ninf_best) { ninf_best = count; patience = 3; }
                    else if (patience > 0) --patience;
                    else all = false;
                    if (++rounds > p.max_rounds) { ++nunconv; done = true; }
                }
                if (done) {
                    if constexpr (!MERGED) break;
                    finish_pattern(gi, count != 0);
                    if constexpr (PAIR) {
                        int tw = 0;
                        if (tw_pending) {
                            tw = 2;
                            if (count == 0) {
                                const int part = sc & 1;
                                ++sc;
                                const uint64_t vmask = s_vmask[tid < 16 * T ? tid : 0] & (has_var ? ~0ULL : 0ULL);
                                const uint64_t gt = (uint64_t)g0 + (unsigned)pair_partner(gi);
                                const int ft = sign_of_var(vmask, gt ^ (gt >> 1));
                                const double fqt = q * (double)(ft > 1 ? 1 : (ft < -1 ? -1 : ft));
                                const bool badt = has_var && (basic ? ((ft == 0) || (fqt < -p.tol)) : (fqt > p.tol));
                                const unsigned long long bt = __ballot(badt);
                                unsigned summt = (unsigned)__popcll(bt);
#pragma unroll
                                for (int sub = 0; sub < 4; ++sub)
                                    if ((bt >> (16 * sub)) & 0xFFFFull) summt |= 0x100u << sub;
                                if (lane == 0 && wave < nwords) { s_inf[part * 8 + wave] = bt; s_sum[part * 8 + wave] = summt; }
                                __syncthreads();
                                STAMP(15);
                                int countt = 0;
                                unsigned tilest = 0;
#pragma unroll
                                for (int w = 0; w < NW; ++w) {
                                    const unsigned sw = (unsigned)__builtin_amdgcn_readfirstlane((int)s_sum[part * 8 + w]);
                                    countt += (int)(sw & 0xFFu);
                                    tilest |= (sw >> 8) << (4 * w);
                                }
                                if (countt == 0) {
                                    record_twin(pair_partner(gi), corner, q, basic);
                                    tw = 0;
                                } else if (countt <= PAIR_MAXC) {
                                    tw = 3;
                                    pr_ncol = 0;
                                    all = true;
                                    tiles = tilest;
                                    soff = part * 8;
                                }
                            }
                        }
                        if (tw == 2) {
                            if (!pair_next(true, f, fn)) break;
                            blocked = false;
                            ninf_best = n + 1; patience = 3; rounds = 0;
                            continue;
                        }
                    }
                    if (!(PAIR && pr_ncol >= 0)) {
                    if constexpr (PAIR) { if (!pair_next(false, f, fn)) break; }
                    else if (++gi >= glen) break;
                    blocked = false;
                    ninf_best = n + 1; patience = 3; rounds = 0;
                    if constexpr (MERGED) {
                        if constexpr (!PAIR) {
                        const uint64_t vmask = s_vmask[tid < 16 * T ? tid : 0] & (has_var ? ~0ULL : 0ULL);
                        const uint64_t gn = (uint64_t)g0 + (unsigned)gi + 1;
                        f = fn;
                        fn = gi + 1 < glen ? sign_of_var(vmask, gn ^ (gn >> 1)) : f;
                        }
                        if (count2 == 0 || p.max_rounds < 1) continue;
                        ninf_best = count2; rounds = 1;
                        all = true;
                        tiles = tiles2;
                        soff += 16;
                    }
                    }
                }
                int single_k = -1;
                if (!all) {
#pragma unroll
                    for (int w = 0; w < NW; ++w) {
                        unsigned long long ww = s_inf[par * 8 + w];
                        ww = ((unsigned long long)(unsigned)__builtin_amdgcn_readfirstlane((int)(ww >> 32)) << 32) |
                             (unsigned)__builtin_amdgcn_readfirstlane((int)ww);
                        if (ww) single_k = (w << 6) + 63 - __builtin_clzll(ww);
                    }
                    tiles = 1u << (single_k >> 4);
                }
                tiles = (unsigned)__builtin_amdgcn_readfirstlane((int)tiles);
                [[maybe_unused]] unsigned tmask = 0;
                if constexpr (LANE_MASKS) {
                    const int tl = lane < T ? lane : 0, wl = tl >> 2, shl = 16 * (tl & 3);
                    tmask = (unsigned)((s_inf[soff + wl] >> shl) & 0xFFFFull) | ((unsigned)((s_bas[par * 8 + wl] >> shl) & 0xFFFFull) << 16);
                }

                [[maybe_unused]] bool chain_end = false;
                while (tiles) {
                    const int kappa = __builtin_ctz(tiles);
                    unsigned pmall, basm;
                    if constexpr (LANE_MASKS) {
                        const unsigned tm = (unsigned)__builtin_amdgcn_readlane((int)tmask, kappa);
                        pmall = tm & 0xFFFFu;
                        if (!all) pmall = 1u << (single_k & 15);
                        basm = tm >> 16;
                    } else {
                        const int wsel = kappa >> 2, sh = 16 * (kappa & 3);
                        pmall = (unsigned)((s_inf[soff + wsel] >> sh) & 0xFFFFull);
                        if (!all) pmall = 1u << (single_k & 15);
                        basm = (unsigned)__builtin_amdgcn_readfirstlane((int)((s_bas[par * 8 + wsel] >> sh) & 0xFFFFull));
                        pmall = (unsigned)__builtin_amdgcn_readfirstlane((int)pmall);
                    }
                    while (pmall) {
                        unsigned rest = 0;
                        if (__builtin_expect(__builtin_popcount(pmall) > MB && !(PAIR && pr_ncol >= 0), 0)) {
                            rest = pmall;
#pragma unroll
                            for (int i = 0; i < MB; ++i) rest &= rest - 1;
                        }
                        const unsigned pm = pmall & ~rest;
                        pmall = rest;
                        const int m = __builtin_popcount(pm);
                        const int bpar = bc & 1;
                        double *P = Pbase + bpar * MB * CW;
                        if constexpr (PAIR) {
                            if (pr_ncol >= 0) P = Pbase + pr_ncol * CW;
                            else ++bc;
                        } else ++bc;
                        int kap = kappa;
                        asm volatile("" : "+s"(kap));
                        STAMP(12);
#define PARTLS_G(i) if constexpr (i < T) { if (__builtin_expect(kap == i, 0)) gather_tile<T, H, W, i>(S, P, a, b, pm); }
                        PARTLS_CASES(PARTLS_G)
#undef PARTLS_G
                        STAMP(13);
                        if (tid < 16 * T && (tid >> 4) == kappa && ((pm >> (tid & 15)) & 1u))
                            P[__builtin_popcount(pm & ((1u << (tid & 15)) - 1u)) * CW + RHSPOS] = q;
                        if constexpr (PAIR) {
                            if (pr_ncol >= 0 && tid < 16 * T && (tid >> 4) == kappa && ((pm >> (tid & 15)) & 1u))
                                s_cpos[pr_ncol + __builtin_popcount(pm & ((1u << (tid & 15)) - 1u))] = basic ? ~mypos : mypos;
                        }
                        int myj = -1;
                        bool my_basic = false;
                        if (rowrho == kappa && rowc < 16 && ((pm >> rowc) & 1u)) {
                            myj = __builtin_popcount(pm & ((1u << rowc) - 1u));
                            my_basic = (basm >> rowc) & 1u;
                        }
                        STAMP(8);
                        __syncthreads();
                        STAMP(1);
                        if (tid == 0) s_veto[bpar ^ 1] = NO_VETO;
                        if (!(PAIR && pr_ncol >= 0)) {
                            int veto;
                            switch (m) {
#define PARTLS_PB(i) case i: if constexpr (i <= MB) veto = panel_block<(i <= MB ? i : 1), CW, MB>(P, Z, U, Dinv, myj, my_basic, p.piv_eps, tid, tid, idle_wave); else veto = 0; break;
                                PARTLS_PB(1) PARTLS_PB(2) PARTLS_PB(3) PARTLS_PB(4) PARTLS_PB(5) PARTLS_PB(6) PARTLS_PB(7) PARTLS_PB(8)
                                PARTLS_PB(9) PARTLS_PB(10) PARTLS_PB(11) PARTLS_PB(12) PARTLS_PB(13) PARTLS_PB(14) PARTLS_PB(15)
#undef PARTLS_PB
                                default: veto = panel_block<MB, CW, MB>(P, Z, U, Dinv, myj, my_basic, p.piv_eps, tid, tid, idle_wave); break;
                            }
                            if (veto < m && tid != RHSPOS) atomicMin(&s_veto[bpar], veto);
                        }
                        STAMP(11);
                        __syncthreads();
                        STAMP(2);
                        const int vs = __builtin_amdgcn_readfirstlane(s_veto[bpar]);
                        unsigned pmx = pm;
                        int mx = m;
                        if (__builtin_expect(vs < m, 0)) {
                            unsigned r = pm;
                            for (int i = 0; i < vs; ++i) r &= r - 1;
                            const unsigned vbit = r & (0u - r);
                            blocked = blocked || (tid == 16 * kappa + __builtin_ctz(vbit));
                            pmall |= pm & ~vbit;
                            pmx = 0;
                            mx = 0;
                            ++nveto;
                        }
                        if constexpr (PAIR) {
                            const bool pr = pr_ncol >= 0;
                            pmx = pr ? 0u : pmx;
                            mx = pr ? 0 : mx;
                            pr_ncol += pr ? m : 0;
                        }
                        bool blk_ok = false;
#pragma unroll PARTLS_UPD_UNROLL
                        for (int s = 0; s < mx; ++s) {
                            const double inv = Dinv[s];
                            blk_ok = blk_ok || (inv != 0.0);
                            const double *Zs = Z + s * CW;
                            double x[L::XN];
#pragma unroll
                            for (int rho = 0; rho < L::XN; ++rho) x[rho] = Zs[a * RS + rho];
#pragma unroll
                            for (int gam = L::GLO; gam < L::GHI; ++gam) {
                                const double yg = -Zs[b * RS + gam] * inv;
#pragma unroll
                                for (int rho = 0; rho <= gam; ++rho)
                                    S[L::idx(rho, gam)] = fma(x[rho], yg, S[L::idx(rho, gam)]);
                            }
                            const double zr = Zs[RHSPOS], zri = zr * inv;
                            if (tid < 16 * T) q = fma(-Zs[mypos], zri, q);
                            corner = fma(-zr, zri, corner);
                        }
                        STAMP(3);
#define PARTLS_F(i) if constexpr (i < T) { if (__builtin_expect(kap == i, 0)) scatter_tile<T, H, W, i>(S, P, a, b, pmx); }
                        PARTLS_CASES(PARTLS_F)
#undef PARTLS_F
                        if (tid < 16 * T && (tid >> 4) == kappa && ((pmx >> (tid & 15)) & 1u)) {
                            const int j = __builtin_popcount(pmx & ((1u << (tid & 15)) - 1u));
                            q = P[j * CW + RHSPOS];
                            if (Dinv[j] != 0.0) basic = !basic;
                            else blocked = true;
                        }
                        progress = progress || blk_ok;
                        npiv += (unsigned)mx;
                        STAMP(4);
                    }
                    tiles &= tiles - 1;
                if constexpr (PAIR) {
                    if (pr_ncol >= 0 && tiles == 0) {
                        const int m = pr_ncol;
                        pr_ncol = -1;
                        const int part = (sc - 1) & 1;
                        int tidp = tid;
                        asm volatile("" : "+v"(tidp));
                        const int lanep = tidp & 63, wavep = __builtin_amdgcn_readfirstlane(tidp >> 6);
                        __syncthreads();
                        if (H == 0 && wavep == 3) pair_solve<CW>(Pbase, s_cpos, m, lanep, RHSPOS, s_pair);
                        __syncthreads();
                        const bool guard = __builtin_amdgcn_readfirstlane(__double2hiint(s_pair[2 * PAIR_MAXC + 1])) != 0;
                        const unsigned long long cw = s_inf[part * 8 + wavep];
                        const bool in_c = has_var && ((cw >> lanep) & 1ull);
                        double qt = q, cornert = corner;
                        {
                            const int rp = tidp < 16 * T ? (tidp & 15) * RS + (tidp >> 4) : RHSPOS;
                            for (int j = 0; j < m; ++j) {
                                const double aj = s_pair[j];
                                qt = fma(-Pbase[j * CW + rp], aj, qt);
                                cornert = fma(-Pbase[j * CW + RHSPOS], aj, cornert);
                            }
                        }
                        if (in_c) {
                            int rank = __popcll(cw & ((1ull << lanep) - 1ull));
#pragma unroll
                            for (int w = 0; w < NW; ++w)
                                if (w < wavep) rank += __popcll(s_inf[part * 8 + w]);
                            qt = s_pair[PAIR_MAXC + rank];
                        }
                        const bool bt = basic != in_c;
                        const uint64_t vmask = s_vmask[tidp < 16 * T ? tidp : 0] & (has_var ? ~0ULL : 0ULL);
                        const uint64_t gt = (uint64_t)g0 + (unsigned)pair_partner(gi);
                        const int ft = sign_of_var(vmask, gt ^ (gt >> 1));
                        const double fqt = qt * (double)(ft > 1 ? 1 : (ft < -1 ? -1 : ft));
                        const bool bad2 = has_var && (bt ? ((ft == 0) || (fqt < -p.tol)) : (fqt > p.tol));
                        const unsigned long long b2 = __ballot(bad2);
                        if (lanep == 0) s_tw[wavep] = b2 != 0ull;
                        __syncthreads();
                        int left = guard ? 1 : 0;
#pragma unroll
                        for (int w = 0; w < 8; ++w) left |= s_tw[w];
                        left = __builtin_amdgcn_readfirstlane(left);
                        if (!left) record_twin(pair_partner(gi), cornert, qt, bt);
                        STAMP(14);
                        if (!pair_next(left != 0, f, fn)) chain_end = true;
                        else {
                            blocked = false;
                            ninf_best = n + 1; patience = 3; rounds = 0;
                            if (!left && count2 != 0 && p.max_rounds >= 1) {
                                ninf_best = count2; rounds = 1;
                                all = true;
                                tiles = (unsigned)__builtin_amdgcn_readfirstlane((int)tiles2);
                                soff = par * 8 + 16;
                                const int tl = lanep < T ? lanep : 0, wl = tl >> 2, shl = 16 * (tl & 3);
                                tmask = (unsigned)((s_inf[soff + wl] >> shl) & 0xFFFFull) | ((unsigned)((s_bas[par * 8 + wl] >> shl) & 0xFFFFull) << 16);
                            }
                        }
                    }
                }
                }
                if constexpr (PAIR) {
                    if (chain_end) break;
                }
            }
            if constexpr (!MERGED) {
                finish_pattern(gi, nunconv != nunconv0);
                if (++gi >= glen) break;
            } else break;
        }
        if constexpr (NODE) {
            if (has_var) p.node_sol[(size_t)chain * p.node_ld + tid] = basic ? q : 0.0;
            if (tid == 0) p.node_obj2[chain] = corner;
            if (p.node_dst) {
                double *snap = p.node_dst[chain];
                if (snap && (H == 0 || T > 1)) {
                    tiles_store<L>(snap, S, t8);
                    if (tid < 16 * T) {
                        snap[(size_t)nslots(T) * 256 + tid] = q;
                        reinterpret_cast<int8_t *>(snap + (nslots(T) * 256 + 16 * T + 8))[tid] = basic ? 1 : 0;
                    }
                    if (tid == 0) snap[(size_t)nslots(T) * 256 + 16 * T] = corner;
                }
            }
            if (p.node_tab && (H == 0 || T > 1)) {
                double *tab = p.node_tab + (size_t)chain * (nslots(T) * 256 + 16 * T + 8);
                tiles_store<L>(tab, S, t8);
                if (tid < 16 * T) p.node_basic[(size_t)chain * 16 * T + tid] = basic ? 1 : 0;
            }
        }
    }
    STAMP_FLUSH;
    __syncthreads();
    if (tid == 0) {
        p.best_obj[blockIdx.x] = sqrt(s_best[0]);
        p.best_pat[blockIdx.x] = reinterpret_cast<long long *>(s_best)[1];
        if (p.second_obj) { p.second_obj[blockIdx.x] = sqrt(s_best[2]); p.second_pat[blockIdx.x] = reinterpret_cast<long long *>(s_best)[3]; }
        if (p.n_pivots && npiv) atomicAdd(p.n_pivots, (unsigned long long)npiv);
        if (p.n_unconverged && nunconv) atomicAdd(p.n_unconverged, (unsigned long long)nunconv);
        if (p.n_vetoes && nveto) atomicAdd(p.n_vetoes, (unsigned long long)nveto);
    }
}

__device__ __forceinline__ void batch_select(SweepParams &p)
{
    const int64_t q = blockIdx.y;
    p.T0 += q * p.batch_t0;
    p.tol = p.batch_tol[q];
    const int64_t o = q * p.batch_out;
    p.best_obj += o;
    p.best_pat += o;
    if (p.second_obj) { p.second_obj += o; p.second_pat += o; }
    if (p.n_unconverged) p.n_unconverged += o;
    if (p.n_pivots) p.n_pivots += o;
    if (p.n_vetoes) p.n_vetoes += o;
    if (p.best_sol) p.best_sol += q * (int64_t)gridDim.x * p.node_ld;
}

template <int T, bool NODE, bool MODELS = false, bool BATCH = false, bool PAIRK = false>
__global__ __launch_bounds__(THREADS, 2) void sweep_blk_kernel(SweepParams p)
{
    if constexpr (BATCH) batch_select(p);
    const int half = __builtin_amdgcn_readfirstlane((int)(threadIdx.x >> 8));
    if (half == 0) sweep_body<T, 0, NODE, 2, MODELS, BATCH, PAIRK>(p);
    else sweep_body<T, 1, NODE, 2, MODELS, BATCH, PAIRK>(p);
}
constexpr bool pair_compiled(int T) { return PARTLS_PAIR && PARTLS_MERGED_SCAN && PARTLS_LANE_MASKS && T > MAXT_S && T <= 16; }

#ifndef PARTLS_SMALL_OCC
#define PARTLS_SMALL_OCC(T) ((T) <= 8 ? 3 : 2)
#endif
template <int T, bool NODE, bool MODELS = false, bool BATCH = false>
__global__ __launch_bounds__(256, PARTLS_SMALL_OCC(T)) void sweep_small_kernel(SweepParams p)
{
    if constexpr (BATCH) batch_select(p);
    sweep_body<T, 0, NODE, 1, MODELS, BATCH>(p);
}

__global__ void layout_reg_kernel(const double *__restrict__ Tfull, int n, int T, double *__restrict__ out, int64_t in_stride, int64_t out_stride)
{
    const int64_t q = blockIdx.y;
    const int ld = n + 1;
    const int ns = T * (T + 1) / 2;
    const int idx = blockIdx.x * blockDim.x + threadIdx.x;
    const int tot = ns * 256 + 16 * T + 1;
    if (idx >= tot) return;
    const double *Tq = Tfull + q * in_stride;
    double *oq = out + q * out_stride;
    if (idx < ns * 256) {
        const int s = idx >> 8, t8 = idx & 255, a = t8 & 15, b = t8 >> 4;
        int gam = 0;
        while ((gam + 1) * (gam + 2) / 2 <= s) ++gam;
        const int rho = s - gam * (gam + 1) / 2;
        const int i = 16 * rho + a, j = 16 * gam + b;
        oq[idx] = (i < n && j < n) ? Tq[(size_t)i * ld + j] : ((i == j) ? 1.0 : 0.0);
    } else if (idx < ns * 256 + 16 * T) {
        const int v = idx - ns * 256;
        oq[idx] = (v < n) ? Tq[(size_t)v * ld + n] : 0.0;
    } else {
        oq[idx] = Tq[(size_t)n * ld + n];
    }
}

}

bool sweep_reg_supported(int n) { return n >= 1 && n <= 16 * blk::MAXT; }
int sweep_reg_tiles(int n) { return (n + 15) / 16; }
bool sweep_reg_exports(int T) { return PARTLS_EXPORT_BIG != 0 && T <= blk::EXPORT_MAXT; }
bool sweep_reg_small(int T) { return T <= blk::MAXT_S; }
size_t sweep_reg_t0_doubles(int T) { return (size_t)T * (T + 1) / 2 * 256 + 16 * (size_t)T + 8; }

hipError_t launch_layout_reg_batch(const double *Tfull, int n, int T, int batch, double *T0reg, hipStream_t s)
{
    const int tot = T * (T + 1) / 2 * 256 + 16 * T + 1;
    hipLaunchKernelGGL(blk::layout_reg_kernel, dim3((tot + 255) / 256, batch), dim3(256), 0, s, Tfull, n, T, T0reg,
                       (int64_t)(n + 1) * (n + 1), (int64_t)sweep_reg_t0_doubles(T));
    return hipGetLastError();
}

hipError_t launch_layout_reg(const double *Tfull, int n, int T, double *T0reg, hipStream_t s)
{
    return launch_layout_reg_batch(Tfull, n, T, 1, T0reg, s);
}

template <class R, class F>
static R dispatch_T(int T, R none, F f)
{
    switch (T) {
#ifdef PARTLS_ONLY_T
        case PARTLS_ONLY_T: return f(std::integral_constant<int, PARTLS_ONLY_T>{});
#else
#define PARTLS_L(i) case i + 1: return f(std::integral_constant<int, i + 1>{});
        PARTLS_CASES(PARTLS_L)
#undef PARTLS_L
#endif
        default: return none;
    }
}

template <int T>
static hipError_t launch_blk_batch_T(const SweepParams &p, int grid, int batch, hipStream_t s)
{
    if constexpr (T <= blk::MAXT_S) hipLaunchKernelGGL((blk::sweep_small_kernel<T, false, false, true>), dim3(grid, batch), dim3(256), 0, s, p);
    else hipLaunchKernelGGL((blk::sweep_blk_kernel<T, false, false, true>), dim3(grid, batch), dim3(blk::THREADS), 0, s, p);
    return hipGetLastError();
}

hipError_t launch_sweep_blk_batch(const SweepParams &p, int T, int grid, int batch, hipStream_t s)
{
    if (p.node_code || batch < 1 || batch > 65535) return hipErrorInvalidValue;
    return dispatch_T(T, hipErrorInvalidValue, [&](auto t) { return launch_blk_batch_T<decltype(t)::value>(p, grid, batch, s); });
}

template <int T>
static hipError_t launch_blk_T(const SweepParams &p, int grid, hipStream_t s, bool models)
{
    if constexpr (T <= blk::MAXT_S) {
        if (p.node_code) hipLaunchKernelGGL((blk::sweep_small_kernel<T, true>), dim3(grid), dim3(256), 0, s, p);
        else if (models) hipLaunchKernelGGL((blk::sweep_small_kernel<T, false, true>), dim3(grid), dim3(256), 0, s, p);
        else hipLaunchKernelGGL((blk::sweep_small_kernel<T, false>), dim3(grid), dim3(256), 0, s, p);
    } else {
        if (p.node_code) hipLaunchKernelGGL((blk::sweep_blk_kernel<T, true>), dim3(grid), dim3(blk::THREADS), 0, s, p);
        else if (models) hipLaunchKernelGGL((blk::sweep_blk_kernel<T, false, true>), dim3(grid), dim3(blk::THREADS), 0, s, p);
        else if (blk::pair_compiled(T) && p.pair) hipLaunchKernelGGL((blk::sweep_blk_kernel<T, false, false, false, blk::pair_compiled(T)>), dim3(grid), dim3(blk::THREADS), 0, s, p);
        else hipLaunchKernelGGL((blk::sweep_blk_kernel<T, false>), dim3(grid), dim3(blk::THREADS), 0, s, p);
    }
    return hipGetLastError();
}

template <int T>
static int concurrency_T()
{
    if constexpr (T <= blk::MAXT_S) {
        int n = 0;
        if (hipOccupancyMaxActiveBlocksPerMultiprocessor(&n, reinterpret_cast<const void *>(&blk::sweep_small_kernel<T, false>), 256, 0) != hipSuccess || n < 1) n = 1;
        return n;
    }
    return 1;
}
int sweep_reg_concurrency_query(int T);
int sweep_reg_concurrency(int T)
{
    static std::atomic<int> cached[blk::MAXT + 2];
    if (T >= 0 && T <= blk::MAXT) { const int v = cached[T].load(std::memory_order_relaxed); if (v > 0) return v; }
    const int v = sweep_reg_concurrency_query(T);
    if (T >= 0 && T <= blk::MAXT) cached[T].store(v, std::memory_order_relaxed);
    return v;
}
int sweep_reg_concurrency_query(int T)
{
    return dispatch_T(T, 1, [](auto t) { return concurrency_T<decltype(t)::value>(); });
}

hipError_t launch_sweep_blk(const SweepParams &p, int T, int grid, hipStream_t s, bool models)
{
    return dispatch_T(T, hipErrorInvalidValue, [&](auto t) { return launch_blk_T<decltype(t)::value>(p, grid, s, models); });
}

}
```

### partitionedls.jl_amd/csrc/sweep_setup.hip

```cpp
#include "ctx.h"
#include "near_tie.h"
#include "sweep_rules.h"
#include <algorithm>
#include <cmath>
#include <cstring>
#include <numeric>

namespace partls {

SweepParams sweep_params(const partls_ctx *c, bool internal_order)
{
    SweepParams p{};
    const bool permuted = internal_order && !c->order_identity;
    p.n = c->n; p.kbits = c->kbits;
    p.mask = permuted ? c->maskInt.as<uint64_t>() : c->maskTabP;
    p.scratch = c->scratch.as<double>();
    p.tol = c->tol; p.piv_eps = SWEEP_PIV_EPS; p.max_rounds = c->knobs.max_rounds >= 1 ? c->knobs.max_rounds : sweep_max_rounds(c->n);
    for (int k = 0; k < 40; ++k) p.rbit.gbit[k] = (uint8_t)k;
    if (permuted) for (int k = 0; k < c->kbits; ++k) p.rbit.gbit[c->order.gbit[k]] = (uint8_t)k;
    return p;
}

partls_status ensure_sweep_scratch(partls_ctx *c, int grid)
{
    const size_t ld = (size_t)c->n + 1;
    PARTLS_HIP_CHECK(c->scratch.ensure((c->use_reg ? 64 : (size_t)grid * ld * ld) * sizeof(double)));
    return PARTLS_OK;
}

partls_status node_sweep_params(partls_ctx *c, size_t nodes, int64_t chain_len, int grid, SweepParams *p)
{
    const size_t wgs = (size_t)std::max(grid, 4096);
    PARTLS_HIP_CHECK(c->bestObj.ensure(sizeof(double) * wgs));
    PARTLS_HIP_CHECK(c->bestPat.ensure(sizeof(int64_t) * wgs));
    *p = sweep_params(c, false);
    p->g_begin = 0; p->g_end = (int64_t)nodes; p->chain_len = chain_len;
    p->best_obj = c->bestObj.as<double>(); p->best_pat = c->bestPat.as<int64_t>();
    return PARTLS_OK;
}

void bind_sweep_block(SweepParams &p, double *base, int grid, bool runner_up)
{
    const SweepBlock b = sweep_block(base, grid, runner_up);
    bind_counters(p, b.counters);
    p.best_obj = b.best_obj; p.best_pat = b.best_pat;
    p.second_obj = b.second_obj; p.second_pat = b.second_pat;
}

hipError_t launch_any_sweep(partls_ctx *c, SweepParams &p, int grid, bool models)
{
    if (c->use_reg) {
        p.T0 = c->T0reg.as<double>();
        return launch_sweep_blk(p, c->T, grid, c->stream, models);
    }
    p.T0 = c->Tfull.as<double>();
    return c->knobs.eager_generic ? launch_sweep_generic(p, grid, c->stream, models) : launch_sweep_lazy(p, grid, c->stream, models);
}

void opt_codes(const partls_ctx *c, uint64_t pattern, std::vector<int8_t> &codes)
{
    codes.resize((size_t)c->n);
    for (int i = 0; i < c->n; ++i) {
        const int f = sign_of_var(c->mask_tab[(size_t)i], pattern);
        codes[(size_t)i] = (int8_t)((f > 0) - (f < 0));
    }
}

partls_status solve_nodes(partls_ctx *c, const std::vector<int8_t> &codes, size_t cnt, std::vector<double> &sols,
                          std::vector<double> &obj2, unsigned long long *unconv, bool resume, bool want_tab)
{
    c->tab_valid = false;
    const int n = c->n, ld = n + 1;
    sols.assign(cnt * (size_t)n, 0.0);
    obj2.assign(cnt, 0.0);
    if (unconv) *unconv = 0;
    if (cnt == 0) return PARTLS_OK;
    if (codes.size() != cnt * (size_t)n) { set_error("solve_nodes: code array has the wrong size"); return PARTLS_ERR_BAD_ARG; }
    const int grid = (int)std::min<size_t>(cnt, c->use_reg ? 2048 : 512);
    PARTLS_HIP_CHECK(c->nodeCode.ensure(cnt * (size_t)n));
    const size_t out_words = 4 + cnt + cnt * (size_t)n;
    PARTLS_HIP_CHECK(c->nodeSol.ensure(out_words * sizeof(double)));
    const bool coop = !c->use_reg && cnt == 1 && !c->knobs.no_coop && !c->coop_fallback;
    c->coop_fallback = false;
    if (coop) {
        const size_t need = ((size_t)2 * ld * ld + (size_t)n / 8 + 2) * sizeof(double);
        if (c->scratch.bytes < need) c->coop_state_valid = false;
        PARTLS_HIP_CHECK(c->scratch.ensure(need));
    } else {
        c->coop_state_valid = false;
        const partls_status ss = ensure_sweep_scratch(c, grid);
        if (ss != PARTLS_OK) return ss;
    }
    PARTLS_HIP_CHECK(hipMemsetAsync(c->nodeSol.p, 0, 4 * sizeof(unsigned long long), c->stream));
    PARTLS_HIP_CHECK(hipMemcpyAsync(c->nodeCode.p, codes.data(), cnt * (size_t)n, hipMemcpyHostToDevice, c->stream));
    SweepParams p;
    const partls_status ps = node_sweep_params(c, cnt, 1, grid, &p);
    if (ps != PARTLS_OK) return ps;
    bind_counters(p, c->nodeSol.as<unsigned long long>());
    p.node_code = c->nodeCode.as<int8_t>();
    p.node_obj2 = c->nodeSol.as<double>() + 4; p.node_sol = c->nodeSol.as<double>() + 4 + cnt; p.node_ld = n;
    const bool dump_reg = want_tab && cnt == 1 && c->use_reg, dump_coop = want_tab && coop;
    const bool dump = dump_reg || dump_coop;
    const size_t tabd = dump_reg ? sweep_reg_t0_doubles(c->T) : (dump_coop ? (size_t)ld * ld : 0);
    if (dump) {
        if (dump_reg) {
            PARTLS_HIP_CHECK(c->nodeTab.ensure(tabd * sizeof(double)));
            PARTLS_HIP_CHECK(c->nodeBasic.ensure((size_t)16 * c->T));
        }
        if (c->hTabDoubles < tabd) {
            c->hTabDoubles = 0;
            PARTLS_HIP_CHECK(c->hTab.alloc(tabd));
            PARTLS_HIP_CHECK(c->hBasic.alloc(1024 + 16 ));
            c->hTabDoubles = tabd;
        }
        if (dump_reg) { p.node_tab = c->nodeTab.as<double>(); p.node_basic = c->nodeBasic.as<int8_t>(); }
    }
    if (coop) {
        p.T0 = c->Tfull.as<double>();
        p.resume = (resume && c->coop_state_valid) ? 1 : 0;
        PARTLS_HIP_CHECK(c->gridCtr.ensure(64));
        p.grid_ctr = c->gridCtr.as<unsigned>();
        p.coop_fault = c->knobs.coop_fault;
        c->coop_state_valid = false;
        const int rows_wg = c->knobs.coop_rows > 0 ? c->knobs.coop_rows : 6;
        int nwg = (ld + rows_wg - 1) / rows_wg;
        if (nwg > 128) nwg = 128;
        PARTLS_HIP_CHECK(launch_sweep_coop(p, nwg, c->stream));
    } else {
        PARTLS_HIP_CHECK(launch_any_sweep(c, p, grid));
    }
    unsigned long long counters[4] = {0, 0, 0, 0};
    std::vector<double> outw_big;
    double *outw_buf;
    if (out_words <= ((size_t)64 << 20) / sizeof(double)) { PARTLS_HIP_CHECK(c->nodeOut.resize(out_words)); outw_buf = c->nodeOut.data(); }
    else { outw_big.resize(out_words); outw_buf = outw_big.data(); }
    const double *outw = outw_buf;
    PARTLS_HIP_CHECK(hipMemcpyAsync(outw_buf, c->nodeSol.p, out_words * sizeof(double), hipMemcpyDeviceToHost, c->stream));
    if (dump_reg) {
        PARTLS_HIP_CHECK(hipMemcpyAsync(c->hTab, c->nodeTab.p, tabd * sizeof(double), hipMemcpyDeviceToHost, c->stream));
        PARTLS_HIP_CHECK(hipMemcpyAsync(c->hBasic, c->nodeBasic.p, (size_t)16 * c->T, hipMemcpyDeviceToHost, c->stream));
    }
    if (dump_coop) {
        const char *flagbuf = static_cast<const char *>(c->scratch.p) + (size_t)2 * ld * ld * sizeof(double);
        PARTLS_HIP_CHECK(hipMemcpyAsync(c->hBasic, flagbuf, (size_t)n + 1, hipMemcpyDeviceToHost, c->stream));
        PARTLS_HIP_CHECK(hipStreamSynchronize(c->stream));
        const size_t img = (size_t)(c->hBasic[n] & 1) * ld * ld;
        PARTLS_HIP_CHECK(hipMemcpyAsync(c->hTab, c->scratch.as<double>() + img, tabd * sizeof(double), hipMemcpyDeviceToHost, c->stream));
    }
    PARTLS_HIP_CHECK(hipStreamSynchronize(c->stream));
    std::memcpy(counters, outw, sizeof(counters));
    if (coop && (counters[0] >> 40)) {
        c->coop_fallback = true;
        return solve_nodes(c, codes, cnt, sols, obj2, unconv, false, want_tab);
    }
    if (coop) c->coop_state_valid = counters[0] == 0;
    std::copy(outw + 4, outw + 4 + cnt, obj2.begin());
    std::copy(outw + 4 + cnt, outw + out_words, sols.begin());
    if (unconv) *unconv = counters[0];
    c->last_pivots = counters[1]; c->last_vetoes = counters[2]; c->last_blocks = counters[3];
    c->tab_valid = dump && counters[0] == 0;
    c->tab_full = dump_coop;
    return PARTLS_OK;
}

static partls_status nodes_on_stream(partls_ctx *c, const double *T0reg, double tol, size_t cnt, const int8_t *code, double *obj2,
                                     double *sol, unsigned long long *counters, int max_rounds)
{
    c->tab_valid = false;
    c->coop_state_valid = false;
    if (cnt == 0) return PARTLS_OK;
    const int n = c->n;
    const int grid = (int)std::min<size_t>(cnt, c->use_reg ? 2048 : 512);
    SweepParams p;
    partls_status st = ensure_sweep_scratch(c, grid);
    if (st == PARTLS_OK) st = node_sweep_params(c, cnt, 1, grid, &p);
    if (st != PARTLS_OK) return st;
    p.max_rounds = max_rounds;
    bind_counters(p, counters);
    p.node_code = code; p.node_obj2 = obj2; p.node_sol = sol; p.node_ld = n;
    if (T0reg) {
        p.T0 = T0reg; p.tol = tol;
        PARTLS_HIP_CHECK(launch_sweep_blk(p, c->T, grid, c->stream));
    } else {
        PARTLS_HIP_CHECK(launch_any_sweep(c, p, grid));
    }
    return PARTLS_OK;
}

partls_status solve_nodes_device(partls_ctx *c, size_t cnt, const int8_t *code, double *obj2, double *sol,
                                 unsigned long long *counters, int max_rounds)
{
    return nodes_on_stream(c, nullptr, 0.0, cnt, code, obj2, sol, counters, max_rounds);
}

partls_status solve_nodes_device_at(partls_ctx *c, const double *T0reg, double tol, size_t cnt, const int8_t *code, double *obj2,
                                    double *sol, unsigned long long *counters, int max_rounds)
{
    if (!c->use_reg || !T0reg) { set_error("solve_nodes_device_at: needs a register-kernel context and a tableau"); return PARTLS_ERR_STATE; }
    return nodes_on_stream(c, T0reg, tol, cnt, code, obj2, sol, counters, max_rounds);
}

}

using namespace partls;

partls_status partls::calibrate_bit_order(partls_ctx *c)
{
    const int kb = c->kbits, n = c->n;
    c->order_ready = true;
    c->order_identity = true;
    c->flip_cost.clear();
    for (int k = 0; k < 40; ++k) c->order.gbit[k] = (uint8_t)k;
    if (kb < 2 || c->knobs.bit_order == 1) return PARTLS_OK;
    const int ncu = c->ncu;
    const int nseg = kb >= 8 ? 2 : 1;
    const int seg_len = (kb + nseg - 1) / nseg, L = seg_len + 1;
    if (c->knobs.bit_order != 2 && ((int64_t)1 << kb) < (int64_t)ncu * 32 * (8 + seg_len)) return PARTLS_OK;
    const int chains = std::max(ncu - ncu % nseg, 2 * nseg);
    const size_t steps = (size_t)chains * L;

    PARTLS_HIP_CHECK(c->nodeCode.ensure(steps * (size_t)n));
    PARTLS_HIP_CHECK(c->nodePiv.ensure((3 * steps + 8) * sizeof(unsigned)));
    PARTLS_HIP_CHECK(c->nodeSol.ensure((4 + (size_t)chains + (size_t)chains * n) * sizeof(double)));
    SweepParams p;
    partls_status st = ensure_sweep_scratch(c, chains);
    if (st == PARTLS_OK) st = node_sweep_params(c, steps, L, chains, &p);
    if (st != PARTLS_OK) return st;
    PARTLS_HIP_CHECK(hipMemsetAsync(c->nodePiv.p, 0, 8 * sizeof(unsigned), c->stream));
    t_begin(c, PARTLS_T_CALIB);
    PARTLS_HIP_CHECK(launch_walk_codes(c->maskTabP, n, kb, chains, L, seg_len, nseg, c->nodeCode.as<int8_t>(), c->stream));
    p.n_unconverged = c->nodePiv.as<unsigned long long>();
    p.node_code = c->nodeCode.as<int8_t>();
    p.node_obj2 = c->nodeSol.as<double>() + 4; p.node_sol = c->nodeSol.as<double>() + 4 + chains; p.node_ld = n;
    p.node_piv = c->nodePiv.as<unsigned>() + 8;
    PARTLS_HIP_CHECK(launch_any_sweep(c, p, chains));
    t_end(c, PARTLS_T_CALIB);
    std::vector<unsigned> piv(3 * steps + 8);
    PARTLS_HIP_CHECK(hipMemcpyAsync(piv.data(), c->nodePiv.p, (3 * steps + 8) * sizeof(unsigned), hipMemcpyDeviceToHost, c->stream));
    PARTLS_HIP_CHECK(hipStreamSynchronize(c->stream));
    t_collect(c);
    c->coop_state_valid = false;
    c->tab_valid = false;
    unsigned long long unconv = 0;
    std::memcpy(&unconv, piv.data(), sizeof(unconv));
    if (unconv) return PARTLS_OK;

    const double ns = c->use_reg ? 0.5 * c->T * (c->T + 1) : 0.0;
    const double per_pivot = 730.0 + 4.4 * ns;
    const double w_block = c->use_reg ? c->knobs.cal_wb * 4400.0 / per_pivot : 0.0, w_scan = c->use_reg ? c->knobs.cal_ws * 2100.0 / per_pivot : 0.0;
    std::vector<double> cost((size_t)kb, 0.0);
    std::vector<int> cnt((size_t)kb, 0);
    for (int ch = 0; ch < chains; ++ch)
        for (int i = 1; i < L; ++i) {
            const int k = walk_flipped_bit(ch, i, kb, seg_len, nseg);
            const unsigned *now = &piv[8 + 3 * ((size_t)ch * L + i)], *was = now - 3;
            const double scans = (double)(now[2] - was[2]);
            cost[(size_t)k] += (double)(now[0] - was[0]) + w_block * (double)(now[1] - was[1]) + w_scan * (scans > 1.0 ? scans - 1.0 : 0.0);
            ++cnt[(size_t)k];
        }
    for (int k = 0; k < kb; ++k) cost[(size_t)k] = cnt[(size_t)k] ? cost[(size_t)k] / cnt[(size_t)k] : 0.0;
    std::vector<int> by_cost((size_t)kb);
    std::iota(by_cost.begin(), by_cost.end(), 0);
    std::stable_sort(by_cost.begin(), by_cost.end(), [&](int a, int b) { return cost[(size_t)a] < cost[(size_t)b]; });
    c->flip_cost = cost;
    double pred_ref = 0.0, pred_sorted = 0.0, wgt = 0.5;
    for (int b = 0; b < kb; ++b, wgt *= 0.5) { pred_ref += wgt * cost[(size_t)b]; pred_sorted += wgt * cost[(size_t)by_cost[(size_t)b]]; }
    if (c->knobs.bit_order != 2 && !(pred_sorted < 0.98 * pred_ref)) return PARTLS_OK;
    bool ident = true;
    for (int b = 0; b < kb; ++b) { c->order.gbit[by_cost[(size_t)b]] = (uint8_t)b; ident = ident && by_cost[(size_t)b] == b; }
    if (ident) return PARTLS_OK;
    std::vector<uint64_t> mi((size_t)n);
    for (int i = 0; i < n; ++i) {
        uint64_t m = c->mask_tab[(size_t)i], q = 0;
        for (; m; m &= m - 1) q |= 1ULL << c->order.gbit[__builtin_ctzll(m)];
        mi[(size_t)i] = q;
    }
    PARTLS_HIP_CHECK(c->maskInt.ensure((size_t)n * sizeof(uint64_t)));
    PARTLS_HIP_CHECK(hipMemcpyAsync(c->maskInt.p, mi.data(), (size_t)n * sizeof(uint64_t), hipMemcpyHostToDevice, c->stream));
    PARTLS_HIP_CHECK(hipStreamSynchronize(c->stream));
    c->order_identity = false;
    return PARTLS_OK;
}

int64_t partls::reference_pattern(const partls_ctx *c, int64_t q)
{
    if (q < 0 || c->order_identity) return q;
    uint64_t r = 0;
    for (int k = 0; k < c->kbits; ++k) r |= (((uint64_t)q >> c->order.gbit[k]) & 1ULL) << k;
    return (int64_t)r;
}

bool partls::sweep_pairs(const partls_ctx *c, int64_t total)
{
    if (!c->use_reg || sweep_reg_small(c->T) || c->T > 16 || c->knobs.pair == 0) return false;
    if (c->knobs.pair == 1) return true;
    const int kb = c->kbits, seg_len = (kb + (kb >= 8 ? 2 : 1) - 1) / (kb >= 8 ? 2 : 1);
    if (kb < 2 || ((int64_t)1 << kb) < (int64_t)c->ncu * 32 * (8 + seg_len) || total < (int64_t)c->ncu * 32) return false;
    int live = 0;
    for (int k = 0; k < kb; ++k)
        if (c->order.gbit[k] == 0)
            for (int i = 0; i < c->n; ++i) live += ((c->mask_tab[(size_t)i] >> k) & 1ULL) != 0 && c->hScale[(size_t)i] != 0.0;
    return live >= 12 && live <= 16;
}

bool partls::sweep_plan(partls_ctx *c, int64_t total, int64_t *chain_len_out, int *grid_out, const char *who)
{
    int64_t chain_len;
    if (c->knobs.chain_len > 0) chain_len = c->knobs.chain_len;
    else if (c->use_reg) {
        const int ncu = c->ncu;
        const int64_t per_chain = total >= (int64_t)ncu * 2048 * 8 ? 2048 : 1024;
        const int conc = sweep_reg_concurrency(c->T);
        if (conc > 1) {
            const int64_t slots = (int64_t)ncu * conc;
            const int64_t k = std::max<int64_t>(1, (total + slots * per_chain - 1) / (slots * per_chain));
            chain_len = std::max<int64_t>(4, (total + k * slots - 1) / (k * slots));
        } else {
        int64_t k = (total + (int64_t)ncu * per_chain - 1) / ((int64_t)ncu * per_chain);
        if (k < 2) k = 2;
        chain_len = (total + k * ncu - 1) / (k * ncu);
        if (chain_len < 16) chain_len = 16;
        }
    } else {
        const int ncu = c->ncu;
        chain_len = 256;
        while (chain_len > 16 && (total + chain_len - 1) / chain_len < ncu) chain_len >>= 1;
    }
    if (chain_len < 1) chain_len = 1;
    if (c->knobs.chain_len <= 0 && sweep_pairs(c, total)) chain_len += chain_len & 1;
    const int64_t nchains = (total + chain_len - 1) / chain_len;
    if (nchains >= (1LL << 31) || chain_len >= (1LL << 31)) { set_error("%s: more than 2^31 chains in one call; split the Gray-index range", who); return false; }
    int grid = (int)std::min<int64_t>(nchains, c->knobs.grid > 0 ? c->knobs.grid : (c->use_reg ? 4096 : 1024));
    if (grid < 1) grid = 1;
    *chain_len_out = chain_len;
    *grid_out = grid;
    return true;
}

void partls::install_sweep_result(partls_ctx *c, const double *sweep_out, int grid, bool has_sol, double *bobj_out, int64_t *bpat_out)
{
    const SweepBlock b = sweep_block(const_cast<double *>(sweep_out), grid, true);
    c->last_pivots = b.counters[1];
    c->last_vetoes = b.counters[2];
    c->sweep_vetoes = b.counters[2];
    c->export_wg = -1;
    std::vector<int64_t> bp((size_t)grid);
    double bobj = INFINITY;
    int64_t bpat = -1;
    int best_wg = -1;
    for (int i = 0; i < grid; ++i) {
        bp[(size_t)i] = reference_pattern(c, b.best_pat[i]);
        if (bp[(size_t)i] < 0) continue;
        if (bpat < 0 || b.best_obj[i] < bobj || (b.best_obj[i] == bobj && bp[(size_t)i] < bpat)) { bobj = b.best_obj[i]; bpat = bp[(size_t)i]; best_wg = i; }
    }
    if (has_sol) c->export_wg = best_wg;
    c->near_pat.clear();
    c->cand.clear();
    c->near_for = bpat;
    if (bpat >= 0) {
        const double yy = h_reg(c, (int)c->M + 1, (int)c->M + 1);
        const double lim2 = bobj * bobj + c->knobs.near_tie_rel * (yy > 0.0 ? yy : 0.0);
        std::vector<std::pair<double, int64_t>> others;
        for (int i = 0; i < grid; ++i) {
            if (bp[(size_t)i] >= 0) others.emplace_back(b.best_obj[i], bp[(size_t)i]);
            if (b.second_pat[i] >= 0) others.emplace_back(b.second_obj[i], reference_pattern(c, b.second_pat[i]));
        }
        install_near_ties({bobj, bpat}, std::move(others), lim2, 3, c->cand, c->near_pat, c->near_for);
    }
    *bobj_out = bobj;
    *bpat_out = bpat;
}
```

Before: 22.59 million.

## Relayout tableau so pair-twin columns share one tile and solve them directly

Adds a host-side relayout that permutes tableau variables so every variable tied to Gray bit 0 lands in tile slot T-2. The tableau is rebuilt and the interleaved mask is re-uploaded. The twin-pattern check in the pair kernel then gathers that single tile and calls pair_solve on it directly, replacing the earlier route that reused the blocked panel loop with a pr_ncol state machine. This is meant to cut the cross-wave ballot summaries and the extra panel passes per twin. In exchange it adds a one-time re-layout cost, and pairing is now enabled only when that relayout has been applied.

```diff
diff --git a/partitionedls.jl_amd/csrc/ctx.h b/partitionedls.jl_amd/csrc/ctx.h
--- a/partitionedls.jl_amd/csrc/ctx.h
+++ b/partitionedls.jl_amd/csrc/ctx.h
@@ -181,6 +181,8 @@
     std::vector<int> perm;
     std::vector<uint64_t> mask_tab;
     bool use_reg = false;
+    bool pair_laid = false;
+    std::vector<uint64_t> mask_int_host;
     partls::BitOrder order{};
     bool order_ready = false, order_identity = true;
     std::vector<double> flip_cost;
@@ -223,6 +225,7 @@
 partls_status adopt_or_upload(partls_ctx *c, const void *X, int64_t N, int64_t M, int64_t ldX, const double *y, int x_on_device, size_t esz);
 partls_status prepare_weights(partls_ctx *c, const double *w, int64_t N, int on_device);
 partls_status ctx_prepare_tableau(partls_ctx *c);
+partls_status ctx_layout_tableau(partls_ctx *c, bool timed);
 partls_status load_partition(partls_ctx *c, const int64_t *P, int64_t M, int64_t K, int64_t ldP);
 partls_status upload_matrix(partls_ctx *c, void *dst, const void *X, int64_t N, int64_t M, int64_t ldX, size_t esz = sizeof(double));
 constexpr double SWEEP_PIV_EPS = 1e-11;
@@ -243,6 +246,8 @@
 void bind_sweep_block(SweepParams &p, double *base, int grid, bool runner_up);
 hipError_t launch_any_sweep(partls_ctx *c, SweepParams &p, int grid, bool models = false);
 partls_status calibrate_bit_order(partls_ctx *c);
+partls_status prepare_sweep_order(partls_ctx *c);
+partls_status pair_relayout(partls_ctx *c);
 bool sweep_plan(partls_ctx *c, int64_t total, int64_t *chain_len_out, int *grid_out, const char *who);
 bool sweep_pairs(const partls_ctx *c, int64_t total);
 int64_t reference_pattern(const partls_ctx *c, int64_t q);
diff --git a/partitionedls.jl_amd/csrc/opt.hip b/partitionedls.jl_amd/csrc/opt.hip
--- a/partitionedls.jl_amd/csrc/opt.hip
+++ b/partitionedls.jl_amd/csrc/opt.hip
@@ -93,7 +93,7 @@
         return PARTLS_OK;
     }
     if (!c->order_ready) {
-        partls_status st = calibrate_bit_order(c);
+        partls_status st = prepare_sweep_order(c);
         if (st != PARTLS_OK) return st;
     }
     const int n = c->n;
@@ -358,7 +358,7 @@
     *empty = g_begin == g_end;
     if (*empty) return PARTLS_OK;
     if (!c->order_ready) {
-        partls_status st = calibrate_bit_order(c);
+        partls_status st = prepare_sweep_order(c);
         if (st != PARTLS_OK) return st;
     }
     return PARTLS_OK;
@@ -644,7 +644,7 @@
     PARTLS_HIP_CHECK(hipSetDevice(c->device));
     if (cnt == 0) return PARTLS_OK;
     if (!c->order_ready) {
-        partls_status st = calibrate_bit_order(c);
+        partls_status st = prepare_sweep_order(c);
         if (st != PARTLS_OK) return st;
     }
     const int64_t kk = std::min<int64_t>(k, cnt);
@@ -698,7 +698,7 @@
     if (!opt_range_ok(c, "partls_opt_bit_order")) return PARTLS_ERR_UNSUPPORTED;
     PARTLS_HIP_CHECK(hipSetDevice(c->device));
     if (!c->order_ready) {
-        partls_status st = calibrate_bit_order(c);
+        partls_status st = prepare_sweep_order(c);
         if (st != PARTLS_OK) return st;
     }
     for (int k = 0; k < c->kbits; ++k) {
diff --git a/partitionedls.jl_amd/csrc/prepare.hip b/partitionedls.jl_amd/csrc/prepare.hip
--- a/partitionedls.jl_amd/csrc/prepare.hip
+++ b/partitionedls.jl_amd/csrc/prepare.hip
@@ -130,6 +130,7 @@
     c->coop_state_valid = false; c->coop_fallback = false;
     c->tab_valid = false;
     c->order_ready = false; c->order_identity = true; c->flip_cost.clear();
+    c->pair_laid = false;
     c->dw = nullptr; c->ds = nullptr;
     c->x_f32 = false;
     c->last_upload_ms = 0.0; c->last_upload_bytes = 0.0;
@@ -188,18 +189,12 @@
     return ctx_prepare_tableau(c);
 }
 
-partls_status ctx_prepare_tableau(partls_ctx *c)
-{
-    const int64_t M = c->M, K = c->K;
+partls_status ctx_layout_tableau(partls_ctx *c, bool timed)
+{
+    const int64_t M = c->M;
     const double eta = c->eta;
     const bool faithful = c->faithful;
     const uint32_t flags = c->flags;
-    c->n = faithful ? (int)M + 1 : (int)M;
-    c->kbits = faithful ? (int)K + 1 : (int)K;
-    c->perm.resize((size_t)c->n);
-    std::iota(c->perm.begin(), c->perm.end(), 0);
-    auto key = [&](int v) { const uint64_t m = c->mask_aug[(size_t)v]; return m ? __builtin_ctzll(m) : 64; };
-    std::stable_sort(c->perm.begin(), c->perm.end(), [&](int a, int b) { return key(a) < key(b); });
     c->mask_tab.resize((size_t)c->n);
     for (int i = 0; i < c->n; ++i) c->mask_tab[(size_t)i] = c->mask_aug[(size_t)c->perm[(size_t)i]];
 
@@ -216,7 +211,7 @@
     }
     PARTLS_HIP_CHECK(c->scale.ensure((size_t)c->n * sizeof(double)));
     PARTLS_HIP_CHECK(c->Tfull.ensure((size_t)(c->n + 1) * (c->n + 1) * sizeof(double)));
-    t_begin(c, PARTLS_T_PREP);
+    if (timed) t_begin(c, PARTLS_T_PREP);
     PARTLS_HIP_CHECK(launch_prep(c->G.as<double>(), c->ldg, (int)M, eta, c->maskAugD.as<uint64_t>(), faithful ? 0 : 1,
                                  c->permP, c->scale.as<double>(), c->Tfull.as<double>(), c->n, c->stream));
     c->use_reg = sweep_reg_supported(c->n) && c->n <= 16 * c->knobs.reg_maxt && !(flags & PARTLS_OPT_GENERIC_KERNEL);
@@ -225,7 +220,23 @@
         PARTLS_HIP_CHECK(c->T0reg.ensure(sweep_reg_t0_doubles(c->T) * sizeof(double)));
         PARTLS_HIP_CHECK(launch_layout_reg(c->Tfull.as<double>(), c->n, c->T, c->T0reg.as<double>(), c->stream));
     }
-    t_end(c, PARTLS_T_PREP);
+    if (timed) t_end(c, PARTLS_T_PREP);
+    return PARTLS_OK;
+}
+
+partls_status ctx_prepare_tableau(partls_ctx *c)
+{
+    const int64_t M = c->M, K = c->K;
+    const bool faithful = c->faithful;
+    c->n = faithful ? (int)M + 1 : (int)M;
+    c->kbits = faithful ? (int)K + 1 : (int)K;
+    c->perm.resize((size_t)c->n);
+    std::iota(c->perm.begin(), c->perm.end(), 0);
+    auto key = [&](int v) { const uint64_t m = c->mask_aug[(size_t)v]; return m ? __builtin_ctzll(m) : 64; };
+    std::stable_sort(c->perm.begin(), c->perm.end(), [&](int a, int b) { return key(a) < key(b); });
+    c->pair_laid = false;
+    partls_status st = ctx_layout_tableau(c, true);
+    if (st != PARTLS_OK) return st;
     PARTLS_HIP_CHECK(c->hG.resize((size_t)c->ldg * c->ldg));
     PARTLS_HIP_CHECK(c->hScale.resize((size_t)c->n));
     PARTLS_HIP_CHECK(hipMemcpyAsync(c->hG.data(), c->G.p, c->hG.size() * sizeof(double), hipMemcpyDeviceToHost, c->stream));
diff --git a/partitionedls.jl_amd/csrc/sweep_blk.hip b/partitionedls.jl_amd/csrc/sweep_blk.hip
--- a/partitionedls.jl_amd/csrc/sweep_blk.hip
+++ b/partitionedls.jl_amd/csrc/sweep_blk.hip
@@ -220,21 +220,23 @@
     return veto;
 }
 
-template <int CW>
+template <int CW, int RS, int KC>
 __device__ __forceinline__ void pair_solve(const double *P, const int *cpos, int m, int lane, int rhspos, double *out)
 {
     const int r = lane & 15, h = lane >> 4;
     const int code = cpos[r < m ? r : 0];
     const unsigned basm = (unsigned)__ballot(code < 0 && lane < m);
-    const int pos = code < 0 ? ~code : code;
+    const int kr = code < 0 ? ~code : code;
+    const int pos = kr * RS + KC;
     double pv[4];
 #pragma unroll
     for (int jj = 0; jj < 4; ++jj) {
         const int c = 4 * h + jj;
-        const double v = P[c * CW + pos];
+        const int cc = cpos[c < m ? c : 0];
+        const double v = P[(cc < 0 ? ~cc : cc) * CW + pos];
         pv[jj] = (r < m && c < m) ? v : 0.0;
     }
-    double qc = P[r * CW + rhspos];
+    double qc = P[kr * CW + rhspos];
     if (r >= m) qc = 0.0;
     bool hard = false;
 #pragma unroll 1
@@ -292,8 +294,9 @@
     [[maybe_unused]] double *const s_pair = U;
     [[maybe_unused]] int *const s_cpos = reinterpret_cast<int *>(Dinv);
     [[maybe_unused]] int *const s_tw = s_cpos + PAIR_MAXC;
+    [[maybe_unused]] int *const s_cm = s_tw + 8;
     static_assert(2 * (MB + 64) >= 2 * PAIR_MAXC + 2, "pair_solve's `out` (doubles) fits U");
-    static_assert(2 * (MB + 64) >= PAIR_MAXC + 8, "s_cpos and s_tw (PAIR_MAXC + 8 ints) fit Dinv (MB + 64 doubles)");
+    static_assert(2 * (MB + 64) >= PAIR_MAXC + 9, "s_cpos, s_tw and s_cm (PAIR_MAXC + 9 ints) fit Dinv (MB + 64 doubles)");
     for (int i = tid; i < 2 * MB * CW; i += THREADS) Pbase[i] = 0.0;
     for (int i = tid; i < MB * CW; i += THREADS) Z[i] = 0.0;
     if (tid < 2 * (MB + 64)) U[tid] = 0.0;
@@ -410,7 +413,6 @@
         };
         int gi = 0;
         [[maybe_unused]] bool tw_pending = false;
-        [[maybe_unused]] int pr_ncol = -1;
         [[maybe_unused]] auto pair_partner = [&](int i) -> int {
             const int j = (((unsigned)g0 + (unsigned)i) & 1u) ? i - 1 : i + 1;
             return (PAIR && j >= 0 && j < glen) ? j : -1;
@@ -533,39 +535,60 @@
                         if (tw_pending) {
                             tw = 2;
                             if (count == 0) {
-                                const int part = sc & 1;
-                                ++sc;
-                                const uint64_t vmask = s_vmask[tid < 16 * T ? tid : 0] & (has_var ? ~0ULL : 0ULL);
+                                constexpr int KC = T - 2, WQ = (16 * KC) >> 6, SHQ = (16 * KC) & 63;
+                                static_assert(KC >= L::G, "the pair column's tile slots all lie in half 1");
+                                int tidp = tid;
+                                asm volatile("" : "+v"(tidp));
+                                const int lanep = tidp & 63, wavep = __builtin_amdgcn_readfirstlane(tidp >> 6), kp = tidp & 15;
+                                const bool mine = (tidp >> 4) == KC;
+                                const uint64_t vmask = s_vmask[tidp < 16 * T ? tidp : 0] & (has_var ? ~0ULL : 0ULL);
                                 const uint64_t gt = (uint64_t)g0 + (unsigned)pair_partner(gi);
                                 const int ft = sign_of_var(vmask, gt ^ (gt >> 1));
-                                const double fqt = q * (double)(ft > 1 ? 1 : (ft < -1 ? -1 : ft));
-                                const bool badt = has_var && (basic ? ((ft == 0) || (fqt < -p.tol)) : (fqt > p.tol));
-                                const unsigned long long bt = __ballot(badt);
-                                unsigned summt = (unsigned)__popcll(bt);
-#pragma unroll
-                                for (int sub = 0; sub < 4; ++sub)
-                                    if ((bt >> (16 * sub)) & 0xFFFFull) summt |= 0x100u << sub;
-                                if (lane == 0 && wave < nwords) { s_inf[part * 8 + wave] = bt; s_sum[part * 8 + wave] = summt; }
+                                gather_tile<T, H, W, KC>(S, Pbase, a, b, 0xFFFFu);
+                                if (mine) Pbase[kp * CW + RHSPOS] = q;
+                                if (H == 0 && wavep == WQ) {
+                                    const double fqt = q * (double)(ft > 1 ? 1 : (ft < -1 ? -1 : ft));
+                                    const bool badt = mine && has_var && (basic ? ((ft == 0) || (fqt < -p.tol)) : (fqt > p.tol));
+                                    const unsigned cmw = (unsigned)(__ballot(badt) >> SHQ) & 0xFFFFu;
+                                    if (badt) s_cpos[__builtin_popcount(cmw & ((1u << kp) - 1u))] = basic ? ~kp : kp;
+                                    if (lanep == 0) s_cm[0] = (int)cmw;
+                                }
                                 __syncthreads();
                                 STAMP(15);
-                                int countt = 0;
-                                unsigned tilest = 0;
-#pragma unroll
-                                for (int w = 0; w < NW; ++w) {
-                                    const unsigned sw = (unsigned)__builtin_amdgcn_readfirstlane((int)s_sum[part * 8 + w]);
-                                    countt += (int)(sw & 0xFFu);
-                                    tilest |= (sw >> 8) << (4 * w);
-                                }
-                                if (countt == 0) {
+                                const unsigned cm = (unsigned)__builtin_amdgcn_readfirstlane(s_cm[0]);
+                                if (cm == 0) {
                                     record_twin(pair_partner(gi), corner, q, basic);
                                     tw = 0;
-                                } else if (countt <= PAIR_MAXC) {
-                                    tw = 3;
-                                    pr_ncol = 0;
-                                    all = true;
-                                    tiles = tilest;
-                                    soff = part * 8;
+                                } else {
+                                    if (H == 0 && wavep == 3) pair_solve<CW, RS, KC>(Pbase, s_cpos, __builtin_popcount(cm), lanep, RHSPOS, s_pair);
+                                    __syncthreads();
+                                    const bool guard = __builtin_amdgcn_readfirstlane(__double2hiint(s_pair[2 * PAIR_MAXC + 1])) != 0;
+                                    const bool in_c = mine && ((cm >> kp) & 1u);
+                                    double qt = q, cornert = corner;
+                                    {
+                                        const int rp = tidp < 16 * T ? kp * RS + (tidp >> 4) : RHSPOS;
+                                        int j = 0;
+                                        for (unsigned mm = cm; mm; mm &= mm - 1u, ++j) {
+                                            const int k = __builtin_ctz(mm);
+                                            const double aj = s_pair[j];
+                                            qt = fma(-Pbase[k * CW + rp], aj, qt);
+                                            cornert = fma(-Pbase[k * CW + RHSPOS], aj, cornert);
+                                        }
+                                    }
+                                    if (in_c) qt = s_pair[PAIR_MAXC + __builtin_popcount(cm & ((1u << kp) - 1u))];
+                                    const bool bt = basic != in_c;
+                                    const double fqt = qt * (double)(ft > 1 ? 1 : (ft < -1 ? -1 : ft));
+                                    const bool bad2 = has_var && (bt ? ((ft == 0) || (fqt < -p.tol)) : (fqt > p.tol));
+                                    const unsigned long long b2 = __ballot(bad2);
+                                    if (lanep == 0) s_tw[wavep] = b2 != 0ull;
+                                    __syncthreads();
+                                    int left = guard ? 1 : 0;
+#pragma unroll
+                                    for (int w = 0; w < 8; ++w) left |= s_tw[w];
+                                    left = __builtin_amdgcn_readfirstlane(left);
+                                    if (!left) { record_twin(pair_partner(gi), cornert, qt, bt); tw = 0; }
                                 }
+                                STAMP(14);
                             }
                         }
                         if (tw == 2) {
@@ -575,7 +598,7 @@
                             continue;
                         }
                     }
-                    if (!(PAIR && pr_ncol >= 0)) {
+                    {
                     if constexpr (PAIR) { if (!pair_next(false, f, fn)) break; }
                     else if (++gi >= glen) break;
                     blocked = false;
@@ -613,7 +636,6 @@
                     tmask = (unsigned)((s_inf[soff + wl] >> shl) & 0xFFFFull) | ((unsigned)((s_bas[par * 8 + wl] >> shl) & 0xFFFFull) << 16);
                 }
 
-                [[maybe_unused]] bool chain_end = false;
                 while (tiles) {
                     const int kappa = __builtin_ctz(tiles);
                     unsigned pmall, basm;
@@ -631,7 +653,7 @@
                     }
                     while (pmall) {
                         unsigned rest = 0;
-                        if (__builtin_expect(__builtin_popcount(pmall) > MB && !(PAIR && pr_ncol >= 0), 0)) {
+                        if (__builtin_expect(__builtin_popcount(pmall) > MB, 0)) {
                             rest = pmall;
 #pragma unroll
                             for (int i = 0; i < MB; ++i) rest &= rest - 1;
@@ -641,10 +663,7 @@
                         const int m = __builtin_popcount(pm);
                         const int bpar = bc & 1;
                         double *P = Pbase + bpar * MB * CW;
-                        if constexpr (PAIR) {
-                            if (pr_ncol >= 0) P = Pbase + pr_ncol * CW;
-                            else ++bc;
-                        } else ++bc;
+                        ++bc;
                         int kap = kappa;
                         asm volatile("" : "+s"(kap));
                         STAMP(12);
@@ -654,10 +673,6 @@
                         STAMP(13);
                         if (tid < 16 * T && (tid >> 4) == kappa && ((pm >> (tid & 15)) & 1u))
                             P[__builtin_popcount(pm & ((1u << (tid & 15)) - 1u)) * CW + RHSPOS] = q;
-                        if constexpr (PAIR) {
-                            if (pr_ncol >= 0 && tid < 16 * T && (tid >> 4) == kappa && ((pm >> (tid & 15)) & 1u))
-                                s_cpos[pr_ncol + __builtin_popcount(pm & ((1u << (tid & 15)) - 1u))] = basic ? ~mypos : mypos;
-                        }
                         int myj = -1;
                         bool my_basic = false;
                         if (rowrho == kappa && rowc < 16 && ((pm >> rowc) & 1u)) {
@@ -668,7 +683,7 @@
                         __syncthreads();
                         STAMP(1);
                         if (tid == 0) s_veto[bpar ^ 1] = NO_VETO;
-                        if (!(PAIR && pr_ncol >= 0)) {
+                        {
                             int veto;
                             switch (m) {
 #define PARTLS_PB(i) case i: if constexpr (i <= MB) veto = panel_block<(i <= MB ? i : 1), CW, MB>(P, Z, U, Dinv, myj, my_basic, p.piv_eps, tid, tid, idle_wave); else veto = 0; break;
@@ -695,12 +710,6 @@
                             mx = 0;
                             ++nveto;
                         }
-                        if constexpr (PAIR) {
-                            const bool pr = pr_ncol >= 0;
-                            pmx = pr ? 0u : pmx;
-                            mx = pr ? 0 : mx;
-                            pr_ncol += pr ? m : 0;
-                        }
                         bool blk_ok = false;
 #pragma unroll PARTLS_UPD_UNROLL
                         for (int s = 0; s < mx; ++s) {
@@ -736,69 +745,6 @@
                         STAMP(4);
                     }
                     tiles &= tiles - 1;
-                if constexpr (PAIR) {
-                    if (pr_ncol >= 0 && tiles == 0) {
-                        const int m = pr_ncol;
-                        pr_ncol = -1;
-                        const int part = (sc - 1) & 1;
-                        int tidp = tid;
-                        asm volatile("" : "+v"(tidp));
-                        const int lanep = tidp & 63, wavep = __builtin_amdgcn_readfirstlane(tidp >> 6);
-                        __syncthreads();
-                        if (H == 0 && wavep == 3) pair_solve<CW>(Pbase, s_cpos, m, lanep, RHSPOS, s_pair);
-                        __syncthreads();
-                        const bool guard = __builtin_amdgcn_readfirstlane(__double2hiint(s_pair[2 * PAIR_MAXC + 1])) != 0;
-                        const unsigned long long cw = s_inf[part * 8 + wavep];
-                        const bool in_c = has_var && ((cw >> lanep) & 1ull);
-                        double qt = q, cornert = corner;
-                        {
-                            const int rp = tidp < 16 * T ? (tidp & 15) * RS + (tidp >> 4) : RHSPOS;
-                            for (int j = 0; j < m; ++j) {
-                                const double aj = s_pair[j];
-                                qt = fma(-Pbase[j * CW + rp], aj, qt);
-                                cornert = fma(-Pbase[j * CW + RHSPOS], aj, cornert);
-                            }
-                        }
-                        if (in_c) {
-                            int rank = __popcll(cw & ((1ull << lanep) - 1ull));
-#pragma unroll
-                            for (int w = 0; w < NW; ++w)
-                                if (w < wavep) rank += __popcll(s_inf[part * 8 + w]);
-                            qt = s_pair[PAIR_MAXC + rank];
-                        }
-                        const bool bt = basic != in_c;
-                        const uint64_t vmask = s_vmask[tidp < 16 * T ? tidp : 0] & (has_var ? ~0ULL : 0ULL);
-                        const uint64_t gt = (uint64_t)g0 + (unsigned)pair_partner(gi);
-                        const int ft = sign_of_var(vmask, gt ^ (gt >> 1));
-                        const double fqt = qt * (double)(ft > 1 ? 1 : (ft < -1 ? -1 : ft));
-                        const bool bad2 = has_var && (bt ? ((ft == 0) || (fqt < -p.tol)) : (fqt > p.tol));
-                        const unsigned long long b2 = __ballot(bad2);
-                        if (lanep == 0) s_tw[wavep] = b2 != 0ull;
-                        __syncthreads();
-                        int left = guard ? 1 : 0;
-#pragma unroll
-                        for (int w = 0; w < 8; ++w) left |= s_tw[w];
-                        left = __builtin_amdgcn_readfirstlane(left);
-                        if (!left) record_twin(pair_partner(gi), cornert, qt, bt);
-                        STAMP(14);
-                        if (!pair_next(left != 0, f, fn)) chain_end = true;
-                        else {
-                            blocked = false;
-                            ninf_best = n + 1; patience = 3; rounds = 0;
-                            if (!left && count2 != 0 && p.max_rounds >= 1) {
-                                ninf_best = count2; rounds = 1;
-                                all = true;
-                                tiles = (unsigned)__builtin_amdgcn_readfirstlane((int)tiles2);
-                                soff = par * 8 + 16;
-                                const int tl = lanep < T ? lanep : 0, wl = tl >> 2, shl = 16 * (tl & 3);
-                                tmask = (unsigned)((s_inf[soff + wl] >> shl) & 0xFFFFull) | ((unsigned)((s_bas[par * 8 + wl] >> shl) & 0xFFFFull) << 16);
-                            }
-                        }
-                    }
-                }
-                }
-                if constexpr (PAIR) {
-                    if (chain_end) break;
                 }
             }
             if constexpr (!MERGED) {
diff --git a/partitionedls.jl_amd/csrc/sweep_setup.hip b/partitionedls.jl_amd/csrc/sweep_setup.hip
--- a/partitionedls.jl_amd/csrc/sweep_setup.hip
+++ b/partitionedls.jl_amd/csrc/sweep_setup.hip
@@ -290,17 +290,66 @@
     return (int64_t)r;
 }
 
-bool partls::sweep_pairs(const partls_ctx *c, int64_t total)
+static bool on_bit0(const partls_ctx *c, int i)
+{
+    if (c->hScale[(size_t)i] == 0.0) return false;
+    for (int k = 0; k < c->kbits; ++k)
+        if (c->order.gbit[k] == 0 && ((c->mask_tab[(size_t)i] >> k) & 1ULL)) return true;
+    return false;
+}
+
+static bool pair_rule(const partls_ctx *c, int64_t total)
 {
     if (!c->use_reg || sweep_reg_small(c->T) || c->T > 16 || c->knobs.pair == 0) return false;
+    int live = 0;
+    for (int i = 0; i < c->n; ++i) live += on_bit0(c, i);
+    if (live > 16) return false;
     if (c->knobs.pair == 1) return true;
     const int kb = c->kbits, seg_len = (kb + (kb >= 8 ? 2 : 1) - 1) / (kb >= 8 ? 2 : 1);
     if (kb < 2 || ((int64_t)1 << kb) < (int64_t)c->ncu * 32 * (8 + seg_len) || total < (int64_t)c->ncu * 32) return false;
-    int live = 0;
-    for (int k = 0; k < kb; ++k)
-        if (c->order.gbit[k] == 0)
-            for (int i = 0; i < c->n; ++i) live += ((c->mask_tab[(size_t)i] >> k) & 1ULL) != 0 && c->hScale[(size_t)i] != 0.0;
-    return live >= 12 && live <= 16;
+    return live >= 12;
+}
+
+bool partls::sweep_pairs(const partls_ctx *c, int64_t total) { return c->pair_laid && pair_rule(c, total); }
+
+partls_status partls::pair_relayout(partls_ctx *c)
+{
+    if (c->pair_laid || !pair_rule(c, (int64_t)1 << c->kbits)) return PARTLS_OK;
+    const int n = c->n, base = 16 * (c->T - 2);
+    std::vector<int> grp, oth, idx;
+    for (int i = 0; i < n; ++i) (on_bit0(c, i) ? grp : oth).push_back(i);
+    idx.assign(oth.begin(), oth.begin() + base);
+    idx.insert(idx.end(), grp.begin(), grp.end());
+    idx.insert(idx.end(), oth.begin() + base, oth.end());
+    c->pair_laid = true;
+    bool same = true;
+    for (int i = 0; i < n; ++i) same = same && idx[(size_t)i] == i;
+    if (same) return PARTLS_OK;
+    std::vector<int> perm((size_t)n);
+    std::vector<double> sc((size_t)n);
+    for (int i = 0; i < n; ++i) { perm[(size_t)i] = c->perm[(size_t)idx[(size_t)i]]; sc[(size_t)i] = c->hScale[(size_t)idx[(size_t)i]]; }
+    c->perm = perm;
+    std::memcpy(c->hScale.data(), sc.data(), (size_t)n * sizeof(double));
+    const partls_status st = ctx_layout_tableau(c, false);
+    if (st != PARTLS_OK) return st;
+    if (!c->order_identity) {
+        c->mask_int_host.resize((size_t)n);
+        for (int i = 0; i < n; ++i) {
+            uint64_t m = c->mask_tab[(size_t)i], q = 0;
+            for (; m; m &= m - 1) q |= 1ULL << c->order.gbit[__builtin_ctzll(m)];
+            c->mask_int_host[(size_t)i] = q;
+        }
+        PARTLS_HIP_CHECK(hipMemcpyAsync(c->maskInt.p, c->mask_int_host.data(), (size_t)n * sizeof(uint64_t), hipMemcpyHostToDevice, c->stream));
+    }
+    c->coop_state_valid = false;
+    c->tab_valid = false;
+    return PARTLS_OK;
+}
+
+partls_status partls::prepare_sweep_order(partls_ctx *c)
+{
+    const partls_status st = calibrate_bit_order(c);
+    return st != PARTLS_OK ? st : pair_relayout(c);
 }
 
 bool partls::sweep_plan(partls_ctx *c, int64_t total, int64_t *chain_len_out, int *grid_out, const char *who)
```

Measured after the change: 24.97 million, median of 6. 1.11x the previous value.
